# bioscan-ml/clibd

Hardware: AMD Instinct MI355X
Metric: paired samples/sec/step (I+D contrastive), global batch 2048 (higher is better)
Workload: dtype bf16

## Files before the change

clibd_amd/csrc/common.h:

```cpp
#pragma once
#include <hip/hip_runtime.h>
#include <stdint.h>

namespace clibd {

typedef __attribute__((ext_vector_type(8))) short bf16x8;
typedef __attribute__((ext_vector_type(4))) short bf16x4;
typedef __attribute__((ext_vector_type(4))) float f32x4;
typedef __attribute__((ext_vector_type(16))) float f32x16;
typedef __attribute__((address_space(3))) void lds_void;
typedef __attribute__((address_space(1))) const void gbl_cvoid;

__device__ __forceinline__ unsigned short f2bf(float x) {
    __bf16 h = (__bf16)x;
    return __builtin_bit_cast(unsigned short, h);
}
__device__ __forceinline__ float bf2f(unsigned short h) {
    return __builtin_bit_cast(float, ((unsigned)h) << 16);
}
__device__ __forceinline__ unsigned pack2bf(float lo, float hi) {
    typedef __bf16 bf16x2_t __attribute__((ext_vector_type(2)));
    typedef float f32x2_t __attribute__((ext_vector_type(2)));
    const bf16x2_t r = __builtin_convertvector((f32x2_t){lo, hi}, bf16x2_t);
    return __builtin_bit_cast(unsigned, r);
}
__device__ __forceinline__ float bfround(float x) { return bf2f(f2bf(x)); }

__device__ __forceinline__ unsigned pack4fp8(float a, float b, float c, float d) {
    a = __builtin_amdgcn_fmed3f(a, -448.f, 448.f); b = __builtin_amdgcn_fmed3f(b, -448.f, 448.f);
    c = __builtin_amdgcn_fmed3f(c, -448.f, 448.f); d = __builtin_amdgcn_fmed3f(d, -448.f, 448.f);
    int w = __builtin_amdgcn_cvt_pk_fp8_f32(a, b, 0, false);
    w = __builtin_amdgcn_cvt_pk_fp8_f32(c, d, w, true);
    return (unsigned)w;
}
__device__ __forceinline__ uint2 pack8fp8(const float v[8], float s) {
    uint2 o;
    o.x = pack4fp8(v[0] * s, v[1] * s, v[2] * s, v[3] * s);
    o.y = pack4fp8(v[4] * s, v[5] * s, v[6] * s, v[7] * s);
    return o;
}

__device__ __forceinline__ void glds16(const void* gsrc, void* lds_wave_base) {
    __builtin_amdgcn_global_load_lds((gbl_cvoid*)gsrc, (lds_void*)lds_wave_base, 16, 0, 0);
}

__device__ __forceinline__ void store16_stream(void* p, uint4 v) {
#ifdef CLIBD_NT_STORES
    typedef unsigned u32x4_t __attribute__((ext_vector_type(4)));
    __builtin_nontemporal_store((u32x4_t){v.x, v.y, v.z, v.w}, (u32x4_t*)p);
#else
    *(uint4*)p = v;
#endif
}

__device__ __forceinline__ unsigned drop_hash(unsigned seed, unsigned pair) {
    unsigned x = pair ^ seed;
    x ^= x >> 16; x *= 0x7feb352du; x ^= x >> 15; x *= 0x846ca68bu; x ^= x >> 16;
    return x;
}
__device__ __forceinline__ void drop_pair(unsigned seed, unsigned idx_even, unsigned thr16, float scale, float& f0, float& f1) {
    const unsigned h = drop_hash(seed, idx_even >> 1);
    f0 = (h & 0xffffu) >= thr16 ? scale : 0.f;
    f1 = (h >> 16) >= thr16 ? scale : 0.f;
}
__device__ __forceinline__ float drop_one(unsigned seed, unsigned idx, unsigned thr16, float scale) {
    const unsigned h = drop_hash(seed, idx >> 1);
    return (((idx & 1u) ? (h >> 16) : (h & 0xffffu)) >= thr16) ? scale : 0.f;
}

template <int CTRL>
__device__ __forceinline__ float dpp_mov(float v) {
    return __builtin_bit_cast(float, __builtin_amdgcn_update_dpp(0, __builtin_bit_cast(int, v), CTRL, 0xF, 0xF, false));
}
constexpr int DPP_QUAD_XOR1 = 0xB1, DPP_QUAD_XOR2 = 0x4E, DPP_ROW_HALF_MIRROR = 0x141, DPP_ROW_MIRROR = 0x140, DPP_ROW_ROR8 = 0x128;
__device__ __forceinline__ void permlane32_swap(float& a, float& b) {
    asm volatile("s_nop 1\n\tv_permlane32_swap_b32 %0, %1\n\ts_nop 1" : "+v"(a), "+v"(b));
}
__device__ __forceinline__ void permlane16_swap(float& a, float& b) {
    asm volatile("s_nop 1\n\tv_permlane16_swap_b32 %0, %1\n\ts_nop 1" : "+v"(a), "+v"(b));
}
__device__ __forceinline__ float rows4_sum(float v) {
    float a = v, b = v;
    permlane16_swap(a, b);
    v = a + b;
    a = v; b = v;
    permlane32_swap(a, b);
    return a + b;
}
__device__ __forceinline__ float rows4_max(float v) {
    float a = v, b = v;
    permlane16_swap(a, b);
    v = fmaxf(a, b);
    a = v; b = v;
    permlane32_swap(a, b);
    return fmaxf(a, b);
}
__device__ __forceinline__ float wave_sum(float v) {
    v += dpp_mov<DPP_QUAD_XOR1>(v);
    v += dpp_mov<DPP_QUAD_XOR2>(v);
    v += dpp_mov<DPP_ROW_HALF_MIRROR>(v);
    v += dpp_mov<DPP_ROW_MIRROR>(v);
    return rows4_sum(v);
}
__device__ __forceinline__ float wave_max(float v) {
    v = fmaxf(v, dpp_mov<DPP_QUAD_XOR1>(v));
    v = fmaxf(v, dpp_mov<DPP_QUAD_XOR2>(v));
    v = fmaxf(v, dpp_mov<DPP_ROW_HALF_MIRROR>(v));
    v = fmaxf(v, dpp_mov<DPP_ROW_MIRROR>(v));
    return rows4_max(v);
}

__device__ __forceinline__ float fast_erf(float x) {
    float ax = fabsf(x);
    float t = __builtin_amdgcn_rcpf(1.0f + 0.3275911f * ax);
    float y = ((((1.061405429f * t - 1.453152027f) * t + 1.421413741f) * t - 0.284496736f) * t + 0.254829592f) * t;
    float e = __expf(-ax * ax);
    float r = 1.0f - y * e;
    return copysignf(r, x);
}
__device__ __forceinline__ float gelu_f(float x) {
    return 0.5f * x * (1.0f + fast_erf(x * 0.70710678118654752f));
}
__device__ __forceinline__ void gelu_and_grad_f(float x, float& y, float& dy) {
    const float ax = fabsf(x) * 0.70710678118654752f;
    const float t = __builtin_amdgcn_rcpf(1.0f + 0.3275911f * ax);
    const float poly = ((((1.061405429f * t - 1.453152027f) * t + 1.421413741f) * t - 0.284496736f) * t + 0.254829592f) * t;
    const float e = __expf(-ax * ax);
    const float erfv = copysignf(1.0f - poly * e, x);
    const float cdf = 0.5f * (1.0f + erfv);
    y = x * cdf;
    dy = cdf + x * (0.3989422804014327f * e);
}
typedef float f32x2 __attribute__((ext_vector_type(2)));
__device__ __forceinline__ void gelu_and_grad_x2(f32x2 x, f32x2& y, f32x2& dy) {
    constexpr float K = 0.84932180028801907f;
    constexpr float P = 0.3275911f * 0.70710678118654752f / K;
    f32x2 ax = {fabsf(x[0]), fabsf(x[1])};
    ax = ax * K;
    const f32x2 d = ax * P + 1.0f;
    const f32x2 t = {__builtin_amdgcn_rcpf(d[0]), __builtin_amdgcn_rcpf(d[1])};
    const f32x2 poly = ((((0.5307027145f * t - 0.7265760135f) * t + 0.7107068705f) * t - 0.142248368f) * t + 0.127414796f) * t;
    const f32x2 s = ax * ax;
    const f32x2 e = {__builtin_amdgcn_exp2f(-s[0]), __builtin_amdgcn_exp2f(-s[1])};
    const f32x2 h = 0.5f - poly * e;
    const f32x2 hs = {copysignf(h[0], x[0]), copysignf(h[1], x[1])};
    const f32x2 cdf = hs + 0.5f;
    y = x * cdf;
    dy = (x * e) * 0.3989422804014327f + cdf;
}
__device__ __forceinline__ f32x2 bfround2(float a, float b) {
// ... 85 lines not shown
```

clibd_amd/csrc/gemm.hip:

```cpp
#include <stdlib.h>

#include <cmath>

#include "gemm_common.h"
#include "host_util.h"

namespace clibd {

constexpr int BM = 128, BN = 128, BK = 64;
constexpr int TILE_BYTES = BM * BK * 2;
constexpr int GEMM_THREADS = 256;

__device__ __forceinline__ int w_row_perm(int r) {
    const int r6 = r & 63;
    return (r & 64) + w_col_of(r6 >> 4, r6 & 15);
}

__global__ __launch_bounds__(GEMM_THREADS, 2) void gemm_bf16_nt_kernel(GemmParams p) {
    extern __shared__ __attribute__((aligned(16))) char smem[];
    const int tid = threadIdx.x;
    const int lane = tid & 63;
    const int wave = __builtin_amdgcn_readfirstlane(tid >> 6);
    const int wm = wave >> 1, wn = wave & 1;

// ... 25 lines not shown
#pragma unroll
    for (int i = 0; i < 4; ++i)
#pragma unroll
        for (int j = 0; j < 4; ++j) acc[i][j] = (f32x4){0.f, 0.f, 0.f, 0.f};

    const int frow = lane & 15, fch = lane >> 4;
    int a_off[4], w_off[4];
#pragma unroll
    for (int t = 0; t < 4; ++t) {
        const int ra = wm * 64 + t * 16 + frow;
        const int rw = wn * 64 + t * 16 + frow;
        a_off[t] = ra * 128 + ((fch ^ (ra & 7)) << 4);
        w_off[t] = rw * 128 + ((fch ^ (rw & 7)) << 4);
    }

    auto stage = [&](int kt, int buf) {
        char* base = smem + buf * (2 * TILE_BYTES);
        int kta = kt0 + kt;
        if (kta >= p.hole_kt) kta += p.hole_nkt;
        const size_t koff = (size_t)kta * (BK * 2);
#pragma unroll
        for (int j = 0; j < 4; ++j) {
            glds16(a_src[j] + koff, base + (wave * 4 + j) * 1024);
            glds16(w_src[j] + koff, base + TILE_BYTES + (wave * 4 + j) * 1024);
        }
    };

    if (nk > 0) stage(0, 0);
    for (int kt = 0; kt < nk; ++kt) {
        __syncthreads();
        if (kt + 1 < nk) stage(kt + 1, (kt + 1) & 1);
        const char* ab = smem + (kt & 1) * (2 * TILE_BYTES);
        const char* wb = ab + TILE_BYTES;
#pragma unroll
        for (int kk = 0; kk < 2; ++kk) {
            bf16x8 af[4], wf[4];
#pragma unroll
            for (int t = 0; t < 4; ++t) {
                af[t] = *(const bf16x8*)(ab + (a_off[t] ^ (kk << 6)));
                wf[t] = *(const bf16x8*)(wb + (w_off[t] ^ (kk << 6)));
            }
#pragma unroll
            for (int i = 0; i < 4; ++i)
#pragma unroll
                for (int j = 0; j < 4; ++j)
                    acc[i][j] = __builtin_amdgcn_mfma_f32_16x16x32_bf16(wf[j], af[i], acc[i][j], 0, 0, 0);
        }
    }

    const clibd_gemm_epilogue& ep = p.ep;
    if (ep.rank_u != nullptr && split == 0) {
        bf16x8 uf[4], vf[4];
#pragma unroll
        for (int t = 0; t < 4; ++t) {
            uf[t] = (bf16x8){0, 0, 0, 0, 0, 0, 0, 0};
            vf[t] = (bf16x8){0, 0, 0, 0, 0, 0, 0, 0};
            if (fch == 0) {
                const int gm = min(m0 + wm * 64 + t * 16 + frow, p.M - 1);
                const int gn = min(n0 + w_row_perm(wn * 64 + t * 16 + frow), p.N - 1);
                uf[t] = *(const bf16x8*)((const unsigned short*)ep.rank_u + (size_t)gm * ep.ld_rank_u);
                vf[t] = *(const bf16x8*)((const unsigned short*)ep.rank_v + (size_t)gn * 8);
            }
        }
#pragma unroll
        for (int i = 0; i < 4; ++i)
#pragma unroll
            for (int j = 0; j < 4; ++j)
                acc[i][j] = __builtin_amdgcn_mfma_f32_16x16x32_bf16(vf[j], uf[i], acc[i][j], 0, 0, 0);
    }

    const int nb = n0 + wn * 64 + 16 * fch;
    if (nb >= p.N) return;
    float bias[16];
    load_bias16(ep, nb, split == 0, bias);
#pragma unroll
    for (int i = 0; i < 4; ++i) {
        const int m = m0 + wm * 64 + 16 * i + frow;
        if (m >= p.M) continue;
        float v[16];
#pragma unroll
        for (int j = 0; j < 4; ++j)
#pragma unroll
            for (int r = 0; r < 4; ++r) v[4 * j + r] = acc[i][j][r] + bias[4 * j + r];
        store_row16(ep, m, nb, v);
    }
}

__global__ __launch_bounds__(256) void transpose_bf16_kernel(const unsigned short* in, int ld_in, int R, int C,
                                                             unsigned short* out, int ld_out) {
    __shared__ unsigned short tile[64][66];
    const int r0 = blockIdx.y * 64, c0 = blockIdx.x * 64;
    const int tx = threadIdx.x & 63, ty = threadIdx.x >> 6;
    for (int i = ty; i < 64; i += 4) {
        const int r = r0 + i, c = c0 + tx;
        tile[i][tx] = (r < R && c < C) ? in[(size_t)r * ld_in + c] : (unsigned short)0;
    }
    __syncthreads();
    for (int i = ty; i < 64; i += 4) {
        const int c = c0 + i, r = r0 + tx;
        if (c < C && r < ld_out) out[(size_t)c * ld_out + r] = tile[tx][i];
    }
}

__global__ __launch_bounds__(256) void transpose_fp8_bf16_kernel(const unsigned char* __restrict__ in, int ld_in, int R, int C, float scale,
                                                                 unsigned short* __restrict__ out, int ld_out) {
    __shared__ unsigned short tile[64][66];
    const int r0 = blockIdx.y * 64, c0 = blockIdx.x * 64;
    const int tx = threadIdx.x & 63, ty = threadIdx.x >> 6;
    for (int i = ty; i < 64; i += 4) {
        const int r = r0 + i, c = c0 + tx;
        unsigned short v = 0;
        if (r < R && c < C) v = f2bf(__builtin_amdgcn_cvt_f32_fp8((int)in[(size_t)r * ld_in + c], 0) * scale);
        tile[i][tx] = v;
    }
    __syncthreads();
    for (int i = ty; i < 64; i += 4) {
        const int c = c0 + i, r = r0 + tx;
        if (c < C && r < ld_out) out[(size_t)c * ld_out + r] = tile[tx][i];
    }
}

template <int RB>
__global__ __launch_bounds__(256) void transpose_colsum_bf16_kernel(const unsigned short* __restrict__ in, int ld_in, int R, int C,
                                                                    unsigned short* __restrict__ out, int ld_out,
                                                                    float* __restrict__ colsum, float* __restrict__ partials) {
    __shared__ __attribute__((aligned(16))) unsigned short tile[64 * RB * 66];
    const int r0 = blockIdx.y * (64 * RB), c0 = blockIdx.x * 64;
    const int t = threadIdx.x;
    uint4 v[2 * RB];
#pragma unroll
    for (int k = 0; k < 2 * RB; ++k) {
        const int row = (t >> 3) + 32 * k, ch = t & 7;
        v[k] = make_uint4(0u, 0u, 0u, 0u);
        if (r0 + row < R && c0 + 8 * ch < C) v[k] = *(const uint4*)(in + (size_t)(r0 + row) * ld_in + c0 + 8 * ch);
    }
#pragma unroll
    for (int k = 0; k < 2 * RB; ++k) {
        const int row = (t >> 3) + 32 * k, ch = t & 7;
        unsigned* d = (unsigned*)(tile + row * 66 + 8 * ch);
        d[0] = v[k].x; d[1] = v[k].y; d[2] = v[k].z; d[3] = v[k].w;
    }
    __syncthreads();
#pragma unroll
    for (int k = 0; k < 2; ++k) {
        const int c = (t >> 3) + 32 * k, rch = t & 7;
        float sum = 0.f;
#pragma unroll
        for (int rb = 0; rb < RB; ++rb) {
            unsigned short e[8];
#pragma unroll
            for (int j = 0; j < 8; ++j) e[j] = tile[(64 * rb + 8 * rch + j) * 66 + c];
            if (c0 + c < C && r0 + 64 * rb + 8 * rch < ld_out) {
                uint4 o;
                o.x = (unsigned)e[0] | ((unsigned)e[1] << 16); o.y = (unsigned)e[2] | ((unsigned)e[3] << 16);
                o.z = (unsigned)e[4] | ((unsigned)e[5] << 16); o.w = (unsigned)e[6] | ((unsigned)e[7] << 16);
                *(uint4*)(out + (size_t)(c0 + c) * ld_out + r0 + 64 * rb + 8 * rch) = o;
            }
            if (colsum != nullptr) {
#pragma unroll
                for (int j = 0; j < 8; ++j) sum += bf2f(e[j]);
            }
        }
        if (colsum != nullptr) {
            sum += dpp_mov<DPP_QUAD_XOR1>(sum);
            sum += dpp_mov<DPP_QUAD_XOR2>(sum);
            sum += dpp_mov<DPP_ROW_HALF_MIRROR>(sum);
            if (rch == 0 && c0 + c < C) {
// ... 35 lines not shown
            for (int k = 0; k < 8; ++k) v[k] = partials[(size_t)(b + k) * C + c];
#pragma unroll
            for (int k = 0; k < 8; ++k) s += v[k];
        }
        for (; b < b1; ++b) s += partials[(size_t)b * C + c];
    }
    part[w][lane] = s;
    __syncthreads();
    if (w == 0 && c < C) {
        float t = part[0][lane];
        for (int k = 1; k < G; ++k) t += part[k][lane];
        if (c < split) out[c] += t;
        else out_b[c - split] += t;
    }
}

int ordered_colsum_launch(const float* partials, int nblk, int C, float* out, int split, float* out_b, hipStream_t stream) {
    if (nblk <= 0 || C <= 0) return CLIBD_OK;
    const int G = nblk < 16 ? nblk : 16;
    hipLaunchKernelGGL(ordered_colsum_kernel, dim3((unsigned)((C + 63) / 64)), dim3(64 * G), 0, stream, partials, nblk, C, out, split, out_b);
    return check_launch("ordered_colsum");
}

__global__ __launch_bounds__(256) void cast_f32_bf16_kernel(const float* in, unsigned short* out, size_t n) {
    size_t i = ((size_t)blockIdx.x * blockDim.x + threadIdx.x) * 4;
    const size_t stride = (size_t)gridDim.x * blockDim.x * 4;
    for (; i + 3 < n; i += stride) {
        const f32x4 v = *(const f32x4*)(in + i);
        uint2 o;
        o.x = pack2bf(v[0], v[1]);
        o.y = pack2bf(v[2], v[3]);
        *(uint2*)(out + i) = o;
    }
    if (blockIdx.x == 0 && threadIdx.x == 0)
        for (size_t j = n & ~(size_t)3; j < n; ++j) out[j] = f2bf(in[j]);
}

__global__ __launch_bounds__(256) void cast_transpose_f32_bf16_kernel(const float* in, int R, int C,
                                                                      unsigned short* out) {
    __shared__ float tile[64][65];
    const int r0 = blockIdx.y * 64, c0 = blockIdx.x * 64;
    const int tx = threadIdx.x & 63, ty = threadIdx.x >> 6;
    for (int i = ty; i < 64; i += 4) {
        const int r = r0 + i, c = c0 + tx;
        tile[i][tx] = (r < R && c < C) ? in[(size_t)r * C + c] : 0.f;
    }
    __syncthreads();
    for (int i = ty; i < 64; i += 4) {
        const int c = c0 + i, r = r0 + tx;
        if (c < C && r < R) out[(size_t)c * R + r] = f2bf(tile[tx][i]);
    }
}

}

using namespace clibd;

static int gemm_impl(const void* A, int lda, const void* W, int ldw, int M, int N, int K, int hole_k0, int hole_len,
                     const clibd_gemm_epilogue* ep, void* tail_ws, size_t tail_ws_bytes, void* stream) {
    if (!A || !W || !ep) return set_error(CLIBD_EINVAL, "gemm: null pointer");
    if (hole_len < 0 || hole_k0 < 0 || hole_k0 % BK || hole_len % BK || hole_k0 + hole_len > K || (hole_len > 0 && hole_len >= K))
        return set_error(CLIBD_EINVAL, "gemm: bad K hole (multiples of 64 inside [0, K))");
    if (M <= 0 || N <= 0 || K <= 0) return set_error(CLIBD_EINVAL, "gemm: non-positive shape");
    if (K % BK != 0) return set_error(CLIBD_EINVAL, "gemm: K must be a multiple of 64");
    if (N % 16 != 0) return set_error(CLIBD_EINVAL, "gemm: N must be a multiple of 16");
    if (lda % 8 != 0 || ldw % 8 != 0 || lda < K || ldw < K) return set_error(CLIBD_EINVAL, "gemm: bad lda/ldw");
    if (!aligned16(A) || !aligned16(W)) return set_error(CLIBD_EINVAL, "gemm: operands must be 16-byte aligned");
    if (!ep->out_bf16 && !ep->out_f32 && !ep->out_pre_bf16) return set_error(CLIBD_EINVAL, "gemm: no output");
    if ((ep->rank_u == nullptr) != (ep->rank_v == nullptr)) return set_error(CLIBD_EINVAL, "gemm: rank_u/rank_v");
    if (ep->rank_u && (ep->ld_rank_u < 8 || ep->ld_rank_u % 8)) return set_error(CLIBD_EINVAL, "gemm: ld_rank_u");
    if ((ep->act == CLIBD_ACT_GELU_GRAD || ep->act == CLIBD_ACT_MUL_AUX || ep->act == CLIBD_ACT_ADD_AUX) &&
        (!ep->aux_bf16 || ep->ld_aux % 8 || ep->ld_aux < N))
        return set_error(CLIBD_EINVAL, "gemm: GELU_GRAD / MUL_AUX / ADD_AUX need aux_bf16 with ld_aux >= N, % 8");
    if (ep->act == CLIBD_ACT_MUL_AUX_U8 && (!ep->aux_bf16 || ep->ld_aux % 16 || ep->ld_aux < N))
        return set_error(CLIBD_EINVAL, "gemm: MUL_AUX_U8 needs aux (one byte per element) with ld_aux >= N, % 16");
    const bool e12 = ep->act == CLIBD_ACT_GELU_SAVE_GRAD_E12 || ep->act == CLIBD_ACT_MUL_AUX_E12;
    if (e12 && (N % 8 != 0)) return set_error(CLIBD_EINVAL, "gemm: the e4m7 gelu' forms need N % 8 == 0");
    if (ep->act == CLIBD_ACT_MUL_AUX_E12 && (!ep->aux_bf16 || ep->ld_aux % 4 || ep->ld_aux < 3 * (N / 2)))
        return set_error(CLIBD_EINVAL, "gemm: MUL_AUX_E12 needs aux (1.5 bytes per element) with ld_aux >= 3N/2 bytes, % 4");
    if (ep->act == CLIBD_ACT_GELU_SAVE_GRAD_E12 && (!ep->out_pre_bf16 || ep->ld_pre % 4 || ep->ld_pre < 3 * (N / 2)))
        return set_error(CLIBD_EINVAL, "gemm: GELU_SAVE_GRAD_E12 needs out_pre (1.5 bytes per element) with ld_pre >= 3N/2 bytes, % 4");
    if ((ep->act == CLIBD_ACT_GELU_SAVE_GRAD || ep->act == CLIBD_ACT_GELU_SAVE_GRAD_U8) && !ep->out_pre_bf16)
        return set_error(CLIBD_EINVAL, "gemm: GELU_SAVE_GRAD needs out_pre_bf16");
    if (ep->act < 0 || ep->act > CLIBD_ACT_MUL_AUX_E12) return set_error(CLIBD_EINVAL, "gemm: bad act");
    if (ep->residual_f32 && (ep->ld_res % 4 || ep->ld_res < N)) return set_error(CLIBD_EINVAL, "gemm: ld_res");
    if (ep->out_pre_bf16 && (ep->ld_pre % (ep->act == CLIBD_ACT_GELU_SAVE_GRAD_U8 ? 16 : 8) || ep->ld_pre < N)) return set_error(CLIBD_EINVAL, "gemm: ld_pre");
    if (ep->out_bf16 && (ep->ld_out_bf16 % 8 || ep->ld_out_bf16 < N)) return set_error(CLIBD_EINVAL, "gemm: ld_out_bf16");
    if (ep->out_f32 && (ep->ld_out_f32 % 4 || ep->ld_out_f32 < N)) return set_error(CLIBD_EINVAL, "gemm: ld_out_f32");
    if (ep->drop_thr16 < 0 || ep->drop_thr16 > 65535 || (ep->drop_thr16 > 0 && (ep->drop_ld < N || (ep->drop_ld & 1) || ep->split_k > 1)))
        return set_error(CLIBD_EINVAL, "gemm: bad dropout parameters");
    const int split = ep->split_k < 1 ? 1 : ep->split_k;
    if (split > 1 && (ep->out_bf16 || ep->out_pre_bf16 || ep->act != CLIBD_ACT_NONE || ep->residual_f32 || !ep->out_f32))
        return set_error(CLIBD_EINVAL, "gemm: split_k > 1 supports only a plain fp32 accumulate output");
    const void* ptrs[] = {ep->bias, ep->rank_u, ep->rank_v, ep->aux_bf16, ep->residual_f32, ep->out_pre_bf16,
                          ep->out_bf16, ep->out_f32};
    for (const void* q : ptrs)
        if (q && !aligned16(q)) return set_error(CLIBD_EINVAL, "gemm: epilogue pointers must be 16-byte aligned");

    GemmParams p{};
    p.A = (const unsigned short*)A; p.W = (const unsigned short*)W;
    p.M = M; p.N = N; p.K = K; p.lda = lda; p.ldw = ldw;
    p.tiles_m = (M + BM - 1) / BM;
    p.tiles_n = (N + BN - 1) / BN;
    const int ktiles = (K - hole_len) / BK;
    p.ktiles_per_split = (ktiles + split - 1) / split;
    p.ep = *ep;
    p.ep.split_k = split;
    p.splits = 1; p.nk_split = 0; p.split_stride = 0;
    p.hole_kt = hole_len > 0 ? hole_k0 / BK : 0x7fffffff;
    p.hole_nkt = hole_len / BK;
    const size_t tail_need = gemm256_tail_workspace_bytes(M, N, K);
    if (int e = check_workspace("gemm", "tail workspace", tail_ws, tail_ws_bytes, tail_need, "clibd_gemm_tail_workspace_bytes")) return e;
    if (tail_ws != nullptr && tail_need > 0) {
        p.sk_flags = (unsigned*)tail_ws;
        p.sk_ws = (float*)((char*)tail_ws + 1024);
    }
    static const int forced = [] { const char* e = getenv("CLIBD_GEMM_KERNEL"); return e ? atoi(e) : 0; }();
    const bool fold_epi = ep->row_sums != nullptr || ep->row_stats != nullptr;
    if (fold_epi) {
        if (epilogue_kind(p.ep) < 0)
            return set_error(CLIBD_EINVAL, "gemm: LN-fold epilogue: row_sums needs bias + residual_f32 + out_f32 + out_bf16 (act NONE); row_stats needs "
                                           "col_sum_w + bias + GELU_SAVE_GRAD with out_pre_bf16 + out_bf16; no rank update, dropout or split-K");
        if ((ep->row_sums && !aligned16(ep->row_sums)) || (ep->row_stats && !aligned16(ep->row_stats)) || (ep->col_sum_w && !aligned16(ep->col_sum_w)))
            return set_error(CLIBD_EINVAL, "gemm: LN-fold epilogue pointers must be 16-byte aligned");
        if (forced == 1 || hole_len != 0 || !gemm256_try_launch(p, (hipStream_t)stream))
            return set_error(CLIBD_EINVAL, "gemm: the LN-fold epilogues exist in the 256x256 kernel only (M >= 1024, N % 256 == 0, K % 128 == 0, >= 128 tiles)");
        return check_launch("gemm256_bf16_nt");
    }
    if (forced != 1 && hole_len == 0 && gemm256_try_launch(p, (hipStream_t)stream)) return check_launch("gemm256_bf16_nt");
    const long long nblocks = (long long)p.tiles_m * p.tiles_n * split;
    if (nblocks > 0x7fffffffLL) return set_error(CLIBD_EINVAL, "gemm: grid too large");
    static const bool attr_ok = [] {
        return hipFuncSetAttribute((const void*)gemm_bf16_nt_kernel, hipFuncAttributeMaxDynamicSharedMemorySize,
                                   4 * TILE_BYTES) == hipSuccess;
    }();
    (void)attr_ok;
    hipLaunchKernelGGL(gemm_bf16_nt_kernel, dim3((unsigned)nblocks), dim3(GEMM_THREADS), 4 * TILE_BYTES,
                       (hipStream_t)stream, p);
    return check_launch("gemm_bf16_nt");
}

extern "C" size_t clibd_gemm_tail_workspace_bytes(int M, int N, int K) { return gemm256_tail_workspace_bytes(M, N, K); }

extern "C" int clibd_gemm_bf16_nt(const void* A, int lda, const void* W, int ldw, int M, int N, int K,
                                  const clibd_gemm_epilogue* ep, void* workspace, size_t workspace_bytes, void* stream) {
    return gemm_impl(A, lda, W, ldw, M, N, K, 0, 0, ep, workspace, workspace_bytes, stream);
}

extern "C" int clibd_gemm_bf16_nt_khole(const void* A, int lda, const void* W, int ldw, int M, int N, int K, int hole_k0, int hole_len,
                                        const clibd_gemm_epilogue* ep, void* stream) {
    return gemm_impl(A, lda, W, ldw, M, N, K, hole_k0, hole_len, ep, nullptr, 0, stream);
}

extern "C" int clibd_gemm_fp8_nt(const void* A, int lda, const void* W, int ldw, int M, int N, int K, const float* col_scale,
                                 float out_fp8_scale, const clibd_gemm_epilogue* ep, void* stream) {
    if (!A || !W || !ep || !col_scale) return set_error(CLIBD_EINVAL, "gemm_fp8: null pointer");
    if (M <= 0 || N <= 0 || K <= 0 || lda < K || ldw < K) return set_error(CLIBD_EINVAL, "gemm_fp8: bad shape");
    if ((lda & 15) || (ldw & 15) || !aligned16(A) || !aligned16(W) || !aligned16(col_scale)) return set_error(CLIBD_EINVAL, "gemm_fp8: alignment (lda, ldw % 16)");
    if (ep->ld_out_bf16 & 7 || ep->ld_out_f32 & 3 || ep->ld_res & 3 || ep->ld_pre & 7 || ep->ld_rank_u & 7)
        return set_error(CLIBD_EINVAL, "gemm_fp8: leading dimensions");
    if ((ep->out_bf16 && !aligned16(ep->out_bf16)) || (ep->out_f32 && !aligned16(ep->out_f32)) || (ep->out_pre_bf16 && !aligned16(ep->out_pre_bf16)) ||
        (ep->residual_f32 && !aligned16(ep->residual_f32)) || (ep->rank_u && !aligned16(ep->rank_u)) || (ep->rank_v && !aligned16(ep->rank_v)) ||
        (ep->bias && !aligned16(ep->bias)))
        return set_error(CLIBD_EINVAL, "gemm_fp8: pointer alignment");
    if ((ep->rank_u == nullptr) != (ep->rank_v == nullptr)) return set_error(CLIBD_EINVAL, "gemm_fp8: rank_u / rank_v must come together");
    GemmParams p{};
    p.A = (const unsigned short*)A; p.W = (const unsigned short*)W;
    p.M = M; p.N = N; p.K = K; p.lda = lda; p.ldw = ldw;
    p.ep = *ep;
    if (p.ep.split_k < 1) p.ep.split_k = 1;
    p.fp8 = 1; p.col_scale = col_scale; p.out_fp8_scale = out_fp8_scale;
    if (!gemm256_fp8_launch(p, (hipStream_t)stream))
        return set_error(CLIBD_EINVAL, "gemm_fp8: shape / epilogue not supported (N % 256, K % 256, K >= 512, bias required; forms: "
                                       "[lora] bias->bf16 | bias->gelu->fp8 + gelu' | bias[->dropout]+residual->f32)");
    return check_launch("gemm256_fp8_nt");
}

extern "C" int clibd_gemm_fp8_dgrad_nt(const void* A, int lda, const void* W, int ldw, int M, int N, int K, const float* col_scale,
                                       const float* a_row_dequant, float out_fp8_scale, const clibd_gemm_epilogue* ep, void* stream) {
    if (!A || !W || !ep || !col_scale) return set_error(CLIBD_EINVAL, "gemm_fp8_dgrad: null pointer");
    if (M <= 0 || N <= 0 || K <= 0 || lda < K || ldw < K) return set_error(CLIBD_EINVAL, "gemm_fp8_dgrad: bad shape");
    if ((lda & 15) || (ldw & 15) || !aligned16(A) || !aligned16(W) || !aligned16(col_scale) || (a_row_dequant && !aligned16(a_row_dequant)))
        return set_error(CLIBD_EINVAL, "gemm_fp8_dgrad: alignment (lda, ldw % 16)");
    if (ep->ld_out_bf16 & 7 || ep->ld_aux & 7) return set_error(CLIBD_EINVAL, "gemm_fp8_dgrad: leading dimensions");
    if (ep->act == CLIBD_ACT_MUL_AUX_U8 && (!ep->aux_bf16 || ep->ld_aux % 16 || ep->ld_aux < N))
        return set_error(CLIBD_EINVAL, "gemm_fp8_dgrad: MUL_AUX_U8 needs aux (one byte per element) with ld_aux >= N, % 16");
    if (!ep->out_bf16 || !aligned16(ep->out_bf16) || (ep->aux_bf16 && !aligned16(ep->aux_bf16))) return set_error(CLIBD_EINVAL, "gemm_fp8_dgrad: out_bf16 / aux alignment");
    if (ep->out_f32 || ep->residual_f32 || ep->bias || ep->rank_u || ep->rank_v || ep->row_sums || ep->row_stats || ep->col_sum_w)
        return set_error(CLIBD_EINVAL, "gemm_fp8_dgrad: only out_bf16 [+ aux_bf16] epilogues");
    const bool mul_form = ep->act == CLIBD_ACT_MUL_AUX || ep->act == CLIBD_ACT_MUL_AUX_U8 || ep->act == CLIBD_ACT_MUL_AUX_E12;
    if (ep->act == CLIBD_ACT_MUL_AUX_E12 && (!ep->aux_bf16 || ep->ld_aux % 4 || ep->ld_aux < 3 * (N / 2)))
        return set_error(CLIBD_EINVAL, "gemm_fp8_dgrad: MUL_AUX_E12 needs aux (1.5 bytes per element) with ld_aux >= 3N/2 bytes, % 4");
    if (ep->out_pre_bf16 && (!mul_form || !a_row_dequant || !aligned16(ep->out_pre_bf16) || (ep->ld_pre & 7) || ep->ld_pre < N))
        return set_error(CLIBD_EINVAL, "gemm_fp8_dgrad: out_pre_bf16 (bf16 copy) comes with MUL_AUX[_U8] and a_row_dequant only; ld_pre >= N, % 8; 16-byte aligned");
    GemmParams p{};
    p.A = (const unsigned short*)A; p.W = (const unsigned short*)W;
    p.M = M; p.N = N; p.K = K; p.lda = lda; p.ldw = ldw;
    p.ep = *ep;
    if (p.ep.split_k < 1) p.ep.split_k = 1;
    p.fp8 = 1; p.col_scale = col_scale; p.out_fp8_scale = out_fp8_scale; p.a_row_dequant = a_row_dequant;
    p.dual_bf16 = (unsigned short*)p.ep.out_pre_bf16; p.ld_dual = p.ep.ld_pre;
// ... 172 lines not shown
```

clibd_amd/csrc/gemm256.hip:

```cpp
#include <cstdlib>
#include "gemm_common.h"
#include "host_util.h"

namespace clibd {

constexpr int T_M = 256, T_N = 256, T_K = 64;
constexpr int HALF_BYTES = 128 * T_K * 2;
constexpr int STAGE_BYTES = 4 * HALF_BYTES;
constexpr int G256_THREADS = 512;
constexpr int G256_LDS = 2 * STAGE_BYTES;
constexpr size_t G256_SK_FLAG_BYTES = 1024;
#ifndef CLIBD_WS_MIN_TILES_N
#define CLIBD_WS_MIN_TILES_N 1
#endif
#ifndef CLIBD_WS_GROUP
#define CLIBD_WS_GROUP 6
#endif
constexpr int G256_WS_MIN_TILES_N = CLIBD_WS_MIN_TILES_N, G256_WS_GROUP = CLIBD_WS_GROUP;

#define CLIBD_WAIT_VMCNT(n) asm volatile("s_waitcnt vmcnt(" #n ")" ::: "memory")

typedef int i32x8 __attribute__((ext_vector_type(8)));
typedef int i32x4 __attribute__((ext_vector_type(4)));
__device__ __forceinline__ i32x8 cat_frag(bf16x8 lo, bf16x8 hi) {
// ... 268 lines not shown
            for (int b = 0; b < 4; ++b)
#pragma unroll
                for (int c = 0; c < 2; ++c)
#pragma unroll
                    for (int d = 0; d < 2; ++d) acc[a][b][c][d] = (f32x4){0.f, 0.f, 0.f, 0.f};

        int kt = 0;
        PHASE_HEAD(0); PHASE_HEAD(1); PHASE_HEAD(2); PHASE_HEAD(3);
        STAMP(1);
        PHASE_HEAD(4); PHASE_HEAD(5);
        PHASE(6, true, 8); PHASE(7, true, 8);
        STAMP(2);
        for (kt = 2; kt < nk - 2; kt += 2) {
            PHASE(0, true, 8); PHASE(1, true, 8); PHASE(2, true, 8); PHASE(3, true, 8);
            PHASE(4, true, 8); PHASE(5, true, 8); PHASE(6, true, 8); PHASE(7, true, 8);
        }
        STAMP(3);
        PHASE(0, true, 8); PHASE(1, true, 8);
        if (has_next) set_sources(next);
        PHASE_TAIL(2, 6); PHASE_TAIL(3, 4); PHASE_TAIL(4, 2); PHASE_TAIL(5, 0); PHASE_TAIL(6, 0); PHASE_TAIL(7, 0);
        if (wm == 0) BARRIER();
        if constexpr (FP8) {
#pragma unroll
            for (int hm = 0; hm < 2; ++hm)
                asm volatile("s_nop 15\n\ts_nop 15"
                             : "+v"(acc[hm][0][0][0]), "+v"(acc[hm][0][0][1]), "+v"(acc[hm][0][1][0]), "+v"(acc[hm][0][1][1]),
                               "+v"(acc[hm][1][0][0]), "+v"(acc[hm][1][0][1]), "+v"(acc[hm][1][1][0]), "+v"(acc[hm][1][1][1]),
                               "+v"(acc[hm][2][0][0]), "+v"(acc[hm][2][0][1]), "+v"(acc[hm][2][1][0]), "+v"(acc[hm][2][1][1]),
                               "+v"(acc[hm][3][0][0]), "+v"(acc[hm][3][0][1]), "+v"(acc[hm][3][1][0]), "+v"(acc[hm][3][1][1])
                             :: "memory");
        }
        STAMP(4);
        if constexpr (SK) {
            if (slot_cur >= 0) {
                const int srow = 64 * wn + 4 * fch, scol = 128 * wm + 8 * frow;
                if (part_cur > 0) {
                    float* outp = p.sk_ws + ((size_t)(part_cur - 1) * (size_t)p.sk_tail + (size_t)slot_cur) * (size_t)(T_M * T_N);
#pragma unroll
                    for (int hn = 0; hn < 2; ++hn)
#pragma unroll
                        for (int n = 0; n < 2; ++n)
#pragma unroll
                            for (int r = 0; r < 4; ++r) {
                                float* o = outp + (size_t)(srow + 32 * hn + 16 * n + r) * T_N + scol;
                                const f32x4 v0 = (f32x4){acc[0][0][hn][n][r], acc[0][1][hn][n][r], acc[0][2][hn][n][r], acc[0][3][hn][n][r]};
                                const f32x4 v1 = (f32x4){acc[1][0][hn][n][r], acc[1][1][hn][n][r], acc[1][2][hn][n][r], acc[1][3][hn][n][r]};
                                asm volatile("global_store_dwordx4 %0, %1, off sc0 sc1\n\tglobal_store_dwordx4 %0, %2, off offset:16 sc0 sc1" :: "v"(o), "v"(v0), "v"(v1) : "memory");
                            }
                    asm volatile("s_waitcnt vmcnt(0)" ::: "memory");
                    BARRIER();
                    if (tid == 0) __hip_atomic_fetch_add(p.sk_flags + slot_cur, 1u, __ATOMIC_RELAXED, __HIP_MEMORY_SCOPE_AGENT);
                    break;
                }
                if (tid == 0) {
                    while (__hip_atomic_load(p.sk_flags + slot_cur, __ATOMIC_RELAXED, __HIP_MEMORY_SCOPE_AGENT) < (unsigned)(p.sk_parts - 1)) __builtin_amdgcn_s_sleep(16);
                    __hip_atomic_store(p.sk_flags + slot_cur, 0u, __ATOMIC_RELAXED, __HIP_MEMORY_SCOPE_AGENT);
                }
                BARRIER();
                for (int q = 1; q < p.sk_parts; ++q) {
                    const float* inp = p.sk_ws + ((size_t)(q - 1) * (size_t)p.sk_tail + (size_t)slot_cur) * (size_t)(T_M * T_N);
#pragma unroll
                    for (int hn = 0; hn < 2; ++hn)
#pragma unroll
                        for (int n = 0; n < 2; ++n) {
                            f32x4 t0[4], t1[4];
#pragma unroll
                            for (int r = 0; r < 4; ++r) {
                                const float* o = inp + (size_t)(srow + 32 * hn + 16 * n + r) * T_N + scol;
                                asm volatile("global_load_dwordx4 %0, %2, off sc0 sc1\n\tglobal_load_dwordx4 %1, %2, off offset:16 sc0 sc1" : "=&v"(t0[r]), "=&v"(t1[r]) : "v"(o) : "memory");
                            }
                            asm volatile("s_waitcnt vmcnt(0)" : "+v"(t0[0]), "+v"(t0[1]), "+v"(t0[2]), "+v"(t0[3]), "+v"(t1[0]), "+v"(t1[1]), "+v"(t1[2]), "+v"(t1[3]));
#pragma unroll
                            for (int r = 0; r < 4; ++r)
#pragma unroll
                                for (int t = 0; t < 4; ++t) { acc[0][t][hn][n][r] += t0[r][t]; acc[1][t][hn][n][r] += t1[r][t]; }
                        }
                }
            }
        }
        int erow = frow, egrp = fch;
        asm volatile("" : "+v"(erow), "+v"(egrp));
        int nb = n0 + 128 * wm + 8 * erow;
        int mb = m0 + 64 * wn + 4 * egrp;
        constexpr bool RES_KIND = (KIND == EPI_RES_F32 || KIND == EPI_RES_F32_DROP || KIND == EPI_RES_F32_COPY);
        constexpr bool TWO_PASS = (epi_aux_kind(KIND) || RES_KIND || KIND == EPI_ROWNORM_GELU);
        constexpr bool PRELOAD_ROWS = TWO_PASS && !LORA && !FP8;
        f32x4 bias_q[2];
        uint4 in_aux[8];
        f32x4 in_res[8][2];
        float2 in_st[8];
        f32x4 col_s[2];
#define GLOAD128(dst, ptr) asm volatile("global_load_dwordx4 %0, %1, off ; EPI_OPERAND_LOAD" : "=&v"(dst) : "v"(ptr) : "memory")
        constexpr bool BIAS_ASM = BIAS && !FP8;
        if constexpr (BIAS_ASM) {
            const float* bp = ep.bias + nb;
            GLOAD128(bias_q[0], bp);
            GLOAD128(bias_q[1], bp + 4);
        }
        if constexpr (PRELOAD_ROWS) {
#pragma unroll
            for (int n = 0; n < 2; ++n)
#pragma unroll
                for (int r = 0; r < 4; ++r) {
                    const int mc = min(mb + 16 * n + r, p.M - 1);
                    if constexpr (KIND == EPI_ROWNORM_GELU) {
                        in_st[4 * n + r] = *(const float2*)(ep.row_stats + (size_t)mc * 2);
                    } else if constexpr (KIND == EPI_MUL_AUX_U8) {
                        const uint2 c8 = *(const uint2*)((const unsigned char*)ep.aux_bf16 + (size_t)mc * ep.ld_aux + nb);
                        in_aux[4 * n + r] = make_uint4(c8.x, c8.y, 0u, 0u);
                    } else if constexpr (KIND == EPI_MUL_AUX_12) {
                        in_aux[4 * n + r] = load_aux12((const unsigned char*)ep.aux_bf16 + (size_t)mc * ep.ld_aux + (nb >> 1) * 3);
                    } else if constexpr (epi_aux_kind(KIND)) {
                        in_aux[4 * n + r] = load_aux16<epi_aux_nt(KIND)>((const unsigned short*)ep.aux_bf16 + (size_t)mc * ep.ld_aux + nb);
                    } else {
                        const f32x4* rs = (const f32x4*)(ep.residual_f32 + (size_t)mc * ep.ld_res + nb);
                        in_res[4 * n + r][0] = rs[0];
                        in_res[4 * n + r][1] = rs[1];
                    }
                }
        }
        if constexpr (KIND == EPI_ROWNORM_GELU) {
            col_s[0] = *(const f32x4*)(ep.col_sum_w + nb);
            col_s[1] = *(const f32x4*)(ep.col_sum_w + nb + 4);
        }
        if (has_next) {
            ISSUE(1, 2, 1); __builtin_amdgcn_sched_barrier(0);
            ISSUE(1, 3, 1); __builtin_amdgcn_sched_barrier(0);
        }
        erow = frow; egrp = fch;
        asm volatile("" : "+v"(erow), "+v"(egrp));
        nb = n0 + 128 * wm + 8 * erow;
        mb = m0 + 64 * wn + 4 * egrp;
#define EPI_TIED_WAIT(N)                                                                                             \
    do {                                                                                                             \
        if constexpr (BIAS_ASM) asm volatile("s_waitcnt vmcnt(" #N ") ; EPI_OPERAND_WAIT" : "+v"(bias_q[0]), "+v"(bias_q[1])); \
    } while (0)
        if constexpr (KIND == EPI_ROWNORM_GELU) {
            if (!has_next) asm volatile("s_waitcnt vmcnt(10)" ::: "memory");
            EPI_TIED_WAIT(14);
        } else if constexpr (PRELOAD_ROWS && epi_aux_kind(KIND)) {
            if (!has_next) asm volatile("s_waitcnt vmcnt(8)" ::: "memory");
            EPI_TIED_WAIT(12);
        } else if constexpr (PRELOAD_ROWS) {
            if (!has_next) asm volatile("s_waitcnt vmcnt(16)" ::: "memory");
            EPI_TIED_WAIT(20);
        } else {
            if (!has_next) asm volatile("s_waitcnt vmcnt(0)" ::: "memory");
            EPI_TIED_WAIT(4);
        }
#undef EPI_TIED_WAIT
#undef GLOAD128
        unsigned rdexp[2][2];
        if constexpr (FP8) {
            const float* csp = p.col_scale + n0 + 128 * wm + 8 * erow;
            const f32x4 c0 = *(const f32x4*)csp, c1 = *(const f32x4*)(csp + 4);
#pragma unroll
            for (int hm = 0; hm < 2; ++hm)
#pragma unroll
                for (int t = 0; t < 4; ++t) {
                    const float c = hm ? c1[t] : c0[t];
#pragma unroll
                    for (int q = 0; q < 4; ++q) acc[hm][t][q >> 1][q & 1] *= c;
                }
            if constexpr (DG == 2) {
#pragma unroll
                for (int hn = 0; hn < 2; ++hn)
#pragma unroll
                    for (int n = 0; n < 2; ++n) {
                        const f32x4 rd = *(const f32x4*)(p.a_row_dequant + min(mb + 32 * hn + 16 * n, p.M - 4));
                        rdexp[hn][n] = ((__float_as_uint(rd[0]) >> 23) & 0xffu) | (((__float_as_uint(rd[1]) >> 23) & 0xffu) << 8) |
                                       (((__float_as_uint(rd[2]) >> 23) & 0xffu) << 16) | (((__float_as_uint(rd[3]) >> 23) & 0xffu) << 24);
                    }
            }
            if constexpr (DG && !epi_mul_aux_kind(KIND)) {
#pragma unroll
                for (int hn = 0; hn < 2; ++hn)
#pragma unroll
                    for (int n = 0; n < 2; ++n) {
                        const f32x4 rd = *(const f32x4*)(p.a_row_dequant + min(mb + 32 * hn + 16 * n, p.M - 4));
#pragma unroll
                        for (int hm = 0; hm < 2; ++hm)
#pragma unroll
                            for (int t = 0; t < 4; ++t) acc[hm][t][hn][n] *= rd;
                    }
            }
        }
        if (LORA) {
            bf16x8 uf[2][2];
#pragma unroll
            for (int hn = 0; hn < 2; ++hn)
#pragma unroll
                for (int n = 0; n < 2; ++n) {
                    uf[hn][n] = (bf16x8){0, 0, 0, 0, 0, 0, 0, 0};
                    if (egrp == 0) {
                        const int gm = min(m0 + 64 * wn + 32 * hn + 16 * n + erow, p.M - 1);
                        uf[hn][n] = *(const bf16x8*)((const unsigned short*)ep.rank_u + (size_t)gm * ep.ld_rank_u);
                    }
                }
#pragma unroll
            for (int hm = 0; hm < 2; ++hm)
#pragma unroll
                for (int t = 0; t < 4; ++t) {
                    bf16x8 vf = (bf16x8){0, 0, 0, 0, 0, 0, 0, 0};
                    if (egrp == 0) {
                        const int gn = nb + 4 * hm + t;
                        vf = *(const bf16x8*)((const unsigned short*)ep.rank_v + (size_t)gn * 8);
                    }
#pragma unroll
                    for (int n = 0; n < 4; ++n)
                        acc[hm][t][n >> 1][n & 1] = __builtin_amdgcn_mfma_f32_16x16x32_bf16(uf[n >> 1][n & 1], vf, acc[hm][t][n >> 1][n & 1], 0, 0, 0);
                }
            __builtin_amdgcn_sched_barrier(0);
        }

        {
            float bias[8];
            if constexpr (BIAS_ASM) {
#pragma unroll
                for (int e = 0; e < 4; ++e) { bias[e] = bias_q[0][e]; bias[4 + e] = bias_q[1][e]; }
            } else if constexpr (BIAS) {
                load_bias8(ep, nb, bias);
                if constexpr (!TWO_PASS) {
#pragma unroll
                    for (int e = 0; e < 8; ++e) asm volatile("" : "+v"(bias[e]));
                }
            }
#define EPV(hm, t) (BIAS ? acc[hm][t][hn][n][r] + bias[4 * (hm) + (t)] : acc[hm][t][hn][n][r])
#define FOR_ROWS_HN(HN0, HN1, ...)                                                                           \
    _Pragma("unroll") for (int hn = (HN0); hn < (HN1); ++hn)                                                 \
        _Pragma("unroll") for (int n = 0; n < 2; ++n)                                                        \
            _Pragma("unroll") for (int r = 0; r < 4; ++r) {                                                  \
                const int m = mb + 32 * hn + 16 * n + r;                                                     \
                __VA_ARGS__                                                                                  \
            }
#define FOR_ROWS(...) FOR_ROWS_HN(0, 2, __VA_ARGS__)
#define PIN_GROUP(hn_)                                                                                       \
    _Pragma("unroll") for (int hm = 0; hm < 2; ++hm)                                                         \
        _Pragma("unroll") for (int t = 0; t < 4; ++t)                                                        \
            _Pragma("unroll") for (int n2 = 0; n2 < 2; ++n2) asm volatile("" : "+v"(acc[hm][t][hn_][n2]))
            if (KIND == EPI_SPLITK_F32) {
                float* outp = ep.out_f32 + (size_t)split_cur * (size_t)p.split_stride;
                FOR_ROWS({
                    if (m < p.M) {
                        f32x4* o = (f32x4*)(outp + (size_t)m * ep.ld_out_f32 + nb);
                        o[0] = (f32x4){acc[0][0][hn][n][r], acc[0][1][hn][n][r], acc[0][2][hn][n][r], acc[0][3][hn][n][r]};
                        o[1] = (f32x4){acc[1][0][hn][n][r], acc[1][1][hn][n][r], acc[1][2][hn][n][r], acc[1][3][hn][n][r]};
                    }
                })
            } else if (TWO_PASS) {
                float cs8[8];
                if constexpr (KIND == EPI_ROWNORM_GELU) {
                    _Pragma("unroll") for (int e = 0; e < 4; ++e) { cs8[e] = col_s[0][e]; cs8[4 + e] = col_s[1][e]; }
                }
                FOR_ROWS_HN(0, 1, {
                    const int mc = min(m, p.M - 1);
                    float v[8];
                    _Pragma("unroll") for (int hm = 0; hm < 2; ++hm)
                        _Pragma("unroll") for (int t = 0; t < 4; ++t) v[4 * hm + t] = (KIND == EPI_ROWNORM_GELU) ? acc[hm][t][hn][n][r] : EPV(hm, t);
                    if constexpr (KIND == EPI_ROWNORM_GELU) fold_rownorm8(v, in_st[4 * n + r].x, in_st[4 * n + r].y, cs8, bias);
                    else if constexpr (PRELOAD_ROWS) fold_row8_in<KIND>(ep, mc, nb, v, in_aux[4 * n + r], in_res[4 * n + r][0], in_res[4 * n + r][1]);
                    else fold_row8<KIND>(ep, mc, nb, v);
                    _Pragma("unroll") for (int hm = 0; hm < 2; ++hm)
                        _Pragma("unroll") for (int t = 0; t < 4; ++t) acc[hm][t][hn][n][r] = v[4 * hm + t];
                })
                PIN_GROUP(0);
                FOR_ROWS_HN(1, 2, {
                    const int mc = min(m, p.M - 1);
                    float v[8];
                    _Pragma("unroll") for (int hm = 0; hm < 2; ++hm)
                        _Pragma("unroll") for (int t = 0; t < 4; ++t) v[4 * hm + t] = (KIND == EPI_ROWNORM_GELU) ? acc[hm][t][hn][n][r] : EPV(hm, t);
                    if constexpr (KIND == EPI_ROWNORM_GELU) {
                        const float2 st = *(const float2*)(ep.row_stats + (size_t)mc * 2);
                        fold_rownorm8(v, st.x, st.y, cs8, bias);
                    } else {
                        fold_row8<KIND>(ep, mc, nb, v);
                    }
                    _Pragma("unroll") for (int hm = 0; hm < 2; ++hm)
                        _Pragma("unroll") for (int t = 0; t < 4; ++t) acc[hm][t][hn][n][r] = v[4 * hm + t];
                })
                PIN_GROUP(1);
                float keep1 = 0.f, keep2 = 0.f;
                FOR_ROWS({
                    if (m < p.M) {
                        float v[8];
                        _Pragma("unroll") for (int hm = 0; hm < 2; ++hm)
                            _Pragma("unroll") for (int t = 0; t < 4; ++t) v[4 * hm + t] = acc[hm][t][hn][n][r];
                        if (KIND == EPI_ROWNORM_GELU) {
                            store_row8<EPI_GELU_SAVE>(ep, m, nb, v);
                        } else if (DG && epi_mul_aux_kind(KIND)) {
                            *(uint2*)((unsigned char*)ep.out_bf16 + (size_t)m * ep.ld_out_bf16 + nb) = pack8fp8(v, p.out_fp8_scale);
                            if constexpr (DG == 2) {
                                const float rdf = __uint_as_float(((rdexp[hn][n] >> (8 * r)) & 0xffu) << 23);
                                float w8[8];
                                _Pragma("unroll") for (int e = 0; e < 8; ++e) w8[e] = v[e] * rdf;
                                *(uint4*)(p.dual_bf16 + (size_t)m * p.ld_dual + nb) = pack8bf(w8);
                            }
                        } else if (epi_aux_kind(KIND)) {
                            *(uint4*)((unsigned short*)ep.out_bf16 + (size_t)m * ep.ld_out_bf16 + nb) = pack8bf(v);
                        } else {
                            f32x4* o = (f32x4*)(ep.out_f32 + (size_t)m * ep.ld_out_f32 + nb);
                            o[0] = (f32x4){v[0], v[1], v[2], v[3]};
                            o[1] = (f32x4){v[4], v[5], v[6], v[7]};
                            if constexpr (KIND == EPI_RES_F32_COPY) {
                                *(uint4*)((unsigned short*)ep.out_bf16 + (size_t)m * ep.ld_out_bf16 + nb) = pack8bf(v);
                                float s1 = ((v[0] + v[1]) + (v[2] + v[3])) + ((v[4] + v[5]) + (v[6] + v[7]));
                                float s2 = 0.f;
                                _Pragma("unroll") for (int e = 0; e < 8; ++e) s2 = fmaf(v[e], v[e], s2);
                                s1 = row16_sum(s1);
                                s2 = row16_sum(s2);
                                if (erow == 8 * hn + 4 * n + r) { keep1 = s1; keep2 = s2; }
                            }
                        }
                    }
                })
                if constexpr (KIND == EPI_RES_F32_COPY) {
                    const int jm = mb + 32 * (erow >> 3) + 16 * ((erow >> 2) & 1) + (erow & 3);
                    const int slice = (n0 >> 7) + wm;
                    if (jm < p.M) *(float2*)(ep.row_sums + ((size_t)slice * (size_t)p.M + (size_t)jm) * 2) = make_float2(keep1, keep2);
                }
            } else {
                FOR_ROWS({
                    if (m < p.M) {
                        float v[8];
                        _Pragma("unroll") for (int hm = 0; hm < 2; ++hm)
                            _Pragma("unroll") for (int t = 0; t < 4; ++t) v[4 * hm + t] = EPV(hm, t);
                        if (FP8 && KIND == EPI_GELU_SAVE) store_row8_gelu_fp8(ep, m, nb, v, p.out_fp8_scale);
                        else store_row8<KIND>(ep, m, nb, v);
                    }
                })
            }
#undef PIN_GROUP
#undef FOR_ROWS_HN
#undef FOR_ROWS
#undef EPV
        }
        STAMP(5);
        if (DIAG) ++tile_i;
        if (!has_next) break;
        allow_case = (m0 + T_M <= p.M) ? stores_case : 0;
        tile = next;
    }
}

template <int KIND, bool LORA, bool BIAS, bool DIAG, bool FP8>
__global__ __launch_bounds__(G256_THREADS) void gemm256_bf16_nt_kernel(GemmParams p, int ntiles, int skew_ticks, long long* stamps) {
    gemm256_body<KIND, LORA, BIAS, DIAG, FP8, 0>(p, ntiles, skew_ticks, stamps);
}
template <int KIND, bool LORA, bool BIAS>
__global__ __launch_bounds__(G256_THREADS) void gemm256_bf16_nt_sk_kernel(GemmParams p, int ntiles, int skew_ticks, long long* stamps) {
    gemm256_body<KIND, LORA, BIAS, false, false, 0, true>(p, ntiles, skew_ticks, stamps);
}
static const void* kernel_ptr_sk(int kind, bool lora, bool bias) {
    switch (kind) {
        case EPI_BF16: return bias ? nullptr : lora ? (const void*)gemm256_bf16_nt_sk_kernel<EPI_BF16, true, false> : (const void*)gemm256_bf16_nt_sk_kernel<EPI_BF16, false, false>;
        case EPI_ADD_AUX: return bias ? nullptr : lora ? (const void*)gemm256_bf16_nt_sk_kernel<EPI_ADD_AUX, true, false> : (const void*)gemm256_bf16_nt_sk_kernel<EPI_ADD_AUX, false, false>;
        case EPI_RES_F32: return (bias && !lora) ? (const void*)gemm256_bf16_nt_sk_kernel<EPI_RES_F32, false, true> : nullptr;
        case EPI_RES_F32_DROP: return (bias && !lora) ? (const void*)gemm256_bf16_nt_sk_kernel<EPI_RES_F32_DROP, false, true> : nullptr;
        default: return nullptr;
    }
}
template <int KIND, int DG = 1>
__global__ __launch_bounds__(G256_THREADS) void gemm256_fp8_dgrad_kernel(GemmParams p, int ntiles, int skew_ticks, long long* stamps) {
    gemm256_body<KIND, false, false, false, true, DG>(p, ntiles, skew_ticks, stamps);
}

#ifdef CLIBD_GEMM_DIAG
static long long* g_stamp_buffer = nullptr;
static int skew_env_value() {
    static const int v = [] { const char* e = getenv("CLIBD_GEMM_SKEW"); return e ? atoi(e) : 0; }();
    return v;
}
static int band_env_value() {
    static const int v = [] { const char* e = getenv("CLIBD_GEMM_BAND"); return e ? atoi(e) : 0; }();
    return v;
}
#define CLIBD_DIAG_KERNEL(KIND) (const void*)gemm256_bf16_nt_kernel<KIND, false, true, true, false>
#else
static constexpr long long* g_stamp_buffer = nullptr;
static int skew_env_value() { return 0; }
static int band_env_value() { return 0; }
#define CLIBD_DIAG_KERNEL(KIND) (const void*)nullptr
#endif

static const void* kernel_ptr(int kind, bool lora, bool bias, bool diag) {
#define K256(KIND)                                                                                                    \
    (diag ? CLIBD_DIAG_KERNEL(KIND)                                                                                   \
          : lora ? (bias ? (const void*)gemm256_bf16_nt_kernel<KIND, true, true, false, false>                        \
                         : (const void*)gemm256_bf16_nt_kernel<KIND, true, false, false, false>)                      \
                 : (bias ? (const void*)gemm256_bf16_nt_kernel<KIND, false, true, false, false>                       \
                         : (const void*)gemm256_bf16_nt_kernel<KIND, false, false, false, false>))
    switch (kind) {
        case EPI_BF16: return K256(EPI_BF16);
        case EPI_GELU_SAVE: return K256(EPI_GELU_SAVE);
        case EPI_GELU: return K256(EPI_GELU);
        case EPI_F32: return K256(EPI_F32);
        case EPI_MUL_AUX: return K256(EPI_MUL_AUX);
        case EPI_ADD_AUX: return K256(EPI_ADD_AUX);
        case EPI_GELU_SAVE_U8: return K256(EPI_GELU_SAVE_U8);
        case EPI_MUL_AUX_U8: return K256(EPI_MUL_AUX_U8);
        case EPI_GELU_SAVE_12: return K256(EPI_GELU_SAVE_12);
        case EPI_MUL_AUX_12: return K256(EPI_MUL_AUX_12);
        case EPI_RES_F32: return K256(EPI_RES_F32);
        case EPI_RES_F32_DROP: return K256(EPI_RES_F32_DROP);
        case EPI_SPLITK_F32: return (const void*)gemm256_bf16_nt_kernel<EPI_SPLITK_F32, false, false, false, false>;
        case EPI_RES_F32_COPY: return (lora || !bias || diag) ? nullptr : (const void*)gemm256_bf16_nt_kernel<EPI_RES_F32_COPY, false, true, false, false>;
        case EPI_ROWNORM_GELU: return (lora || !bias || diag) ? nullptr : (const void*)gemm256_bf16_nt_kernel<EPI_ROWNORM_GELU, false, true, false, false>;
        default: return K256(EPI_GENERIC);
    }
#undef K256
}

static const void* kernel_ptr_fp8(int kind, bool lora) {
    switch (kind) {
        case EPI_BF16: return lora ? (const void*)gemm256_bf16_nt_kernel<EPI_BF16, true, true, false, true>
                                   : (const void*)gemm256_bf16_nt_kernel<EPI_BF16, false, true, false, true>;
        case EPI_GELU_SAVE: return lora ? nullptr : (const void*)gemm256_bf16_nt_kernel<EPI_GELU_SAVE, false, true, false, true>;
        case EPI_RES_F32: return lora ? nullptr : (const void*)gemm256_bf16_nt_kernel<EPI_RES_F32, false, true, false, true>;
        case EPI_RES_F32_DROP: return lora ? nullptr : (const void*)gemm256_bf16_nt_kernel<EPI_RES_F32_DROP, false, true, false, true>;
        default: return nullptr;
    }
}

static int device_cus() {
    static const int num_cus = [] {
        int dev = 0, n = 256;
        if (hipGetDevice(&dev) == hipSuccess) {
            hipDeviceProp_t prop;
            if (hipGetDeviceProperties(&prop, dev) == hipSuccess && prop.multiProcessorCount > 0) n = prop.multiProcessorCount;
        }
        return n;
    }();
    return num_cus;
}

bool gemm256_fp8_launch(const GemmParams& p, hipStream_t stream) {
    const int nk = p.K / 128;
    if (!p.fp8 || p.col_scale == nullptr || p.K % 128 != 0 || nk < 4 || (nk & 1) || p.N % T_N != 0 || p.M < 1 || p.ep.split_k > 1) return false;
    if (p.ep.bias == nullptr) return false;
    if ((unsigned long long)p.M * p.lda >= (1ull << 32) || (unsigned long long)p.N * p.ldw >= (1ull << 32)) return false;
    const int kind = epilogue_kind(p.ep);
    const bool lora = p.ep.rank_u != nullptr;
    const void* fn = kernel_ptr_fp8(kind, lora);
    if (fn == nullptr) return false;
    if ((p.out_fp8_scale > 0.f) != (kind == EPI_GELU_SAVE)) return false;
    static const bool attr_ok = [] {
        bool ok = true;
        for (int k = 0; k < EPI_NUM_KINDS; ++k)
            for (int l = 0; l < 2; ++l) {
                const void* f = kernel_ptr_fp8(k, l != 0);
                if (f != nullptr) ok = ok && hipFuncSetAttribute(f, hipFuncAttributeMaxDynamicSharedMemorySize, G256_LDS) == hipSuccess;
            }
        return ok;
    }();
    if (!attr_ok) return false;
    GemmParams q = p;
    q.tiles_m = (p.M + T_M - 1) / T_M;
    q.tiles_n = p.N / T_N;
    q.splits = 1;
    q.nk_split = nk;
    q.split_stride = 0;
    q.band = q.tiles_n >= G256_WS_MIN_TILES_N ? -G256_WS_GROUP : 4;
    const long long tiles = (long long)q.tiles_m * q.tiles_n;
    const int grid = (int)(tiles < device_cus() ? tiles : device_cus());
    int ntiles_i = (int)tiles, skew = 0;
    long long* stamp = nullptr;
    void* args[] = {(void*)&q, (void*)&ntiles_i, (void*)&skew, (void*)&stamp};
    return hipLaunchKernel(fn, dim3((unsigned)grid), dim3(G256_THREADS), args, G256_LDS, stream) == hipSuccess;
}

bool gemm256_fp8_dgrad_launch(const GemmParams& p, hipStream_t stream) {
    const int nk = p.K / 128;
    if (!p.fp8 || p.col_scale == nullptr || p.K % 128 != 0 || nk < 4 || (nk & 1) || p.N % T_N != 0 || p.M < 4 || (p.M & 3) || p.ep.split_k > 1) return false;
    if (p.ep.bias != nullptr || p.ep.rank_u != nullptr || p.ep.drop_thr16 > 0) return false;
    if ((unsigned long long)p.M * p.lda >= (1ull << 32) || (unsigned long long)p.N * p.ldw >= (1ull << 32)) return false;
    const int kind = epilogue_kind(p.ep);
    const bool dual = p.dual_bf16 != nullptr;
    const void* fn = kind == EPI_BF16 ? (const void*)gemm256_fp8_dgrad_kernel<EPI_BF16>
                   : kind == EPI_MUL_AUX ? (dual ? (const void*)gemm256_fp8_dgrad_kernel<EPI_MUL_AUX, 2> : (const void*)gemm256_fp8_dgrad_kernel<EPI_MUL_AUX>)
                   : kind == EPI_MUL_AUX_U8 ? (dual ? (const void*)gemm256_fp8_dgrad_kernel<EPI_MUL_AUX_U8, 2> : (const void*)gemm256_fp8_dgrad_kernel<EPI_MUL_AUX_U8>)
                   : kind == EPI_MUL_AUX_12 ? (dual ? (const void*)gemm256_fp8_dgrad_kernel<EPI_MUL_AUX_12, 2> : (const void*)gemm256_fp8_dgrad_kernel<EPI_MUL_AUX_12>)
                   : kind == EPI_ADD_AUX ? (const void*)gemm256_fp8_dgrad_kernel<EPI_ADD_AUX> : nullptr;
    if (fn == nullptr) return false;
    const bool mul = epi_mul_aux_kind(kind);
    if ((p.out_fp8_scale > 0.f) != mul) return false;
    if ((!mul || dual) && p.a_row_dequant == nullptr) return false;
    if (dual && (!mul || (p.ld_dual & 7) || p.ld_dual < p.N || ((uintptr_t)p.dual_bf16 & 15))) return false;
    static const bool attr_ok = [] {
        bool ok = hipFuncSetAttribute((const void*)gemm256_fp8_dgrad_kernel<EPI_BF16>, hipFuncAttributeMaxDynamicSharedMemorySize, G256_LDS) == hipSuccess;
        ok = ok && hipFuncSetAttribute((const void*)gemm256_fp8_dgrad_kernel<EPI_MUL_AUX>, hipFuncAttributeMaxDynamicSharedMemorySize, G256_LDS) == hipSuccess;
// ... 156 lines not shown
```

clibd_amd/csrc/gemm_common.h:

```cpp
#pragma once
#include "common.h"
#include "../../include/clibd_hip.h"

namespace clibd {

struct GemmParams {
    const unsigned short* A;
    const unsigned short* W;
    int M, N, K, lda, ldw;
    int tiles_m, tiles_n, ktiles_per_split;
    clibd_gemm_epilogue ep;
    int splits, nk_split;
    long long split_stride;
    int band;
    int hole_kt, hole_nkt;
    int fp8;
    const float* col_scale;
    float out_fp8_scale;
    const float* a_row_dequant;
    unsigned short* dual_bf16;
    int ld_dual;
    int sk_parts, sk_tail, sk_first, sk_nk_part;
    float* sk_ws;
    unsigned* sk_flags;
};

struct SkPlan { int parts, tail, first, nk_part; };
inline SkPlan plan_stream_k_tail(long long tiles, int num_cus, int nk) {
    SkPlan s{0, 0, 0, 0};
    if (tiles <= 0 || num_cus <= 0 || nk < 24 || (nk & 1)) return s;
    const long long full = (tiles / num_cus) * num_cus;
    const int tail = (int)(tiles - full);
    if (tail == 0 || 2 * tail > num_cus) return s;
    int P = num_cus / tail;
    if (P > 4) P = 4;
    for (; P >= 2; --P) {
        int nkp = (nk + P - 1) / P;
        nkp += nkp & 1;
        if (nkp < 4) nkp = 4;
        const int parts = (nk + nkp - 1) / nkp;
        const int last = nk - (parts - 1) * nkp;
        if (parts >= 2 && last >= 4 && (long long)parts * tail <= num_cus) { s.parts = parts; s.tail = tail; s.first = (int)full; s.nk_part = nkp; return s; }
    }
    return s;
}

__device__ __forceinline__ int w_col_of(int t, int i) { return 16 * (i >> 2) + 4 * t + (i & 3); }

__device__ __forceinline__ int tile_off(int row, int chunk) { return row * 128 + ((chunk ^ (row & 7)) << 4); }

__device__ __forceinline__ void tile_coords(int bid, int tiles_m, int tiles_n, int band, int& tile_m, int& tile_n) {
    const int ntiles = tiles_m * tiles_n;
    const int q = ntiles >> 3, r = ntiles & 7;
    const int xcd = bid & 7, idx = bid >> 3;
    bid = (xcd < r ? xcd * (q + 1) : r * (q + 1) + (xcd - r) * q) + idx;
    if (band < 0) {
        const int G = -band;
        const int g = bid / (tiles_m * G);
        const int rem = bid - g * tiles_m * G;
        const int gw = min(G, tiles_n - g * G);
        tile_m = rem / gw;
        tile_n = g * G + rem - tile_m * gw;
        return;
    }
    const int band_id = bid / (band * tiles_n);
    const int band_m0 = band_id * band;
    const int band_h = min(band, tiles_m - band_m0);
    const int in_band = bid - band_id * band * tiles_n;
    tile_m = band_m0 + in_band % band_h;
    tile_n = in_band / band_h;
}

__device__ __forceinline__ void load_bias16(const clibd_gemm_epilogue& ep, int nb, bool on, float bias[16]) {
#pragma unroll
    for (int e = 0; e < 16; ++e) bias[e] = 0.f;
    if (ep.bias != nullptr && on) {
#pragma unroll
        for (int q = 0; q < 4; ++q) {
            const f32x4 b4 = *(const f32x4*)(ep.bias + nb + 4 * q);
            bias[4 * q + 0] = b4[0]; bias[4 * q + 1] = b4[1]; bias[4 * q + 2] = b4[2]; bias[4 * q + 3] = b4[3];
        }
    }
}

__device__ __forceinline__ void store_row16(const clibd_gemm_epilogue& ep, int m, int nb, float v[16]) {
    if (ep.split_k > 1) {
        float* o = ep.out_f32 + (size_t)m * ep.ld_out_f32 + nb;
#pragma unroll
        for (int e = 0; e < 16; ++e) atomicAdd(o + e, v[e]);
        return;
    }
    if (ep.drop_thr16 > 0) {
        const unsigned base = (unsigned)m * (unsigned)ep.drop_ld + (unsigned)nb;
#pragma unroll
        for (int e = 0; e < 16; e += 2) {
            float f0, f1;
            drop_pair(ep.drop_seed, base + e, (unsigned)ep.drop_thr16, ep.drop_scale, f0, f1);
            v[e] *= f0;
            v[e + 1] *= f1;
        }
    }
    if (ep.act == CLIBD_ACT_GELU_SAVE_GRAD_E12) {
        float dg[16];
        gelu_and_grad_rows<16>(v, dg);
        gelu12_row8* o = (gelu12_row8*)((unsigned char*)ep.out_pre_bf16 + (size_t)m * ep.ld_pre + (nb >> 1) * 3);
        o[0] = gelu12_pack8(dg);
        o[1] = gelu12_pack8(dg + 8);
    } else if (ep.act == CLIBD_ACT_GELU_SAVE_GRAD_U8) {
        float dg[16];
        gelu_and_grad_rows<16>(v, dg);
        uint4 c;
        c.x = geluq_pack4(dg[0], dg[1], dg[2], dg[3]);   c.y = geluq_pack4(dg[4], dg[5], dg[6], dg[7]);
        c.z = geluq_pack4(dg[8], dg[9], dg[10], dg[11]); c.w = geluq_pack4(dg[12], dg[13], dg[14], dg[15]);
        store16_stream((unsigned char*)ep.out_pre_bf16 + (size_t)m * ep.ld_pre + nb, c);
    } else if (ep.act == CLIBD_ACT_GELU_SAVE_GRAD) {
        float dg[16];
        gelu_and_grad_rows<16>(v, dg);
        uint4 lo, hi;
        lo.x = pack2bf(dg[0], dg[1]);   lo.y = pack2bf(dg[2], dg[3]);   lo.z = pack2bf(dg[4], dg[5]);   lo.w = pack2bf(dg[6], dg[7]);
        hi.x = pack2bf(dg[8], dg[9]);   hi.y = pack2bf(dg[10], dg[11]); hi.z = pack2bf(dg[12], dg[13]); hi.w = pack2bf(dg[14], dg[15]);
        uint4* o = (uint4*)((unsigned short*)ep.out_pre_bf16 + (size_t)m * ep.ld_pre + nb);
        store16_stream(o, lo); store16_stream(o + 1, hi);
    } else if (ep.out_pre_bf16 != nullptr) {
        uint4 lo, hi;
        lo.x = pack2bf(v[0], v[1]);   lo.y = pack2bf(v[2], v[3]);   lo.z = pack2bf(v[4], v[5]);   lo.w = pack2bf(v[6], v[7]);
        hi.x = pack2bf(v[8], v[9]);   hi.y = pack2bf(v[10], v[11]); hi.z = pack2bf(v[12], v[13]); hi.w = pack2bf(v[14], v[15]);
        uint4* o = (uint4*)((unsigned short*)ep.out_pre_bf16 + (size_t)m * ep.ld_pre + nb);
        store16_stream(o, lo); store16_stream(o + 1, hi);
#pragma unroll
        for (int e = 0; e < 16; ++e) v[e] = bfround(v[e]);
    }
    if (ep.act == CLIBD_ACT_GELU) {
        gelu_rows<16>(v);
    } else if (ep.act == CLIBD_ACT_GELU_GRAD) {
        const uint4* ax = (const uint4*)((const unsigned short*)ep.aux_bf16 + (size_t)m * ep.ld_aux + nb);
        const uint4 x0 = ax[0], x1 = ax[1];
        const unsigned xs[8] = {x0.x, x0.y, x0.z, x0.w, x1.x, x1.y, x1.z, x1.w};
#pragma unroll
        for (int e = 0; e < 8; ++e) {
            v[2 * e] *= gelu_grad_f(bf2f((unsigned short)(xs[e] & 0xffffu)));
            v[2 * e + 1] *= gelu_grad_f(bf2f((unsigned short)(xs[e] >> 16)));
        }
    }
    if (ep.act == CLIBD_ACT_MUL_AUX_E12) {
        const gelu12_row8* ax = (const gelu12_row8*)((const unsigned char*)ep.aux_bf16 + (size_t)m * ep.ld_aux + (nb >> 1) * 3);
        const gelu12_row8 a0 = ax[0], a1 = ax[1];
        float d[16];
        gelu12_unpack8(a0.w0, a0.w1, a0.w2, d);
        gelu12_unpack8(a1.w0, a1.w1, a1.w2, d + 8);
#pragma unroll
        for (int e = 0; e < 16; ++e) v[e] *= d[e];
    }
    if (ep.act == CLIBD_ACT_MUL_AUX_U8) {
        const uint4 c = *(const uint4*)((const unsigned char*)ep.aux_bf16 + (size_t)m * ep.ld_aux + nb);
        const unsigned cs[4] = {c.x, c.y, c.z, c.w};
#pragma unroll
        for (int q = 0; q < 4; ++q) {
            float d[4];
            geluq_unpack4(cs[q], d);
            v[4 * q] *= d[0]; v[4 * q + 1] *= d[1]; v[4 * q + 2] *= d[2]; v[4 * q + 3] *= d[3];
        }
    }
    if (ep.act == CLIBD_ACT_MUL_AUX || ep.act == CLIBD_ACT_ADD_AUX) {
        const uint4* ax = (const uint4*)((const unsigned short*)ep.aux_bf16 + (size_t)m * ep.ld_aux + nb);
        const uint4 x0 = ax[0], x1 = ax[1];
        const unsigned xs[8] = {x0.x, x0.y, x0.z, x0.w, x1.x, x1.y, x1.z, x1.w};
#pragma unroll
        for (int e = 0; e < 8; ++e) {
            const float a0 = bf2f((unsigned short)(xs[e] & 0xffffu)), a1 = bf2f((unsigned short)(xs[e] >> 16));
            if (ep.act == CLIBD_ACT_MUL_AUX) { v[2 * e] *= a0; v[2 * e + 1] *= a1; }
            else { v[2 * e] += a0; v[2 * e + 1] += a1; }
        }
    }
    if (ep.residual_f32 != nullptr) {
        const f32x4* rs = (const f32x4*)(ep.residual_f32 + (size_t)m * ep.ld_res + nb);
#pragma unroll
        for (int q = 0; q < 4; ++q) {
            const f32x4 r4 = rs[q];
            v[4 * q + 0] += r4[0]; v[4 * q + 1] += r4[1]; v[4 * q + 2] += r4[2]; v[4 * q + 3] += r4[3];
        }
    }
    if (ep.out_f32 != nullptr) {
        f32x4* o = (f32x4*)(ep.out_f32 + (size_t)m * ep.ld_out_f32 + nb);
#pragma unroll
        for (int q = 0; q < 4; ++q) store16_stream(o + q, __builtin_bit_cast(uint4, (f32x4){v[4 * q], v[4 * q + 1], v[4 * q + 2], v[4 * q + 3]}));
    }
    if (ep.out_bf16 != nullptr) {
        uint4 lo, hi;
        lo.x = pack2bf(v[0], v[1]);   lo.y = pack2bf(v[2], v[3]);   lo.z = pack2bf(v[4], v[5]);   lo.w = pack2bf(v[6], v[7]);
        hi.x = pack2bf(v[8], v[9]);   hi.y = pack2bf(v[10], v[11]); hi.z = pack2bf(v[12], v[13]); hi.w = pack2bf(v[14], v[15]);
        uint4* o = (uint4*)((unsigned short*)ep.out_bf16 + (size_t)m * ep.ld_out_bf16 + nb);
        store16_stream(o, lo); store16_stream(o + 1, hi);
    }
}

__device__ __forceinline__ void load_bias8(const clibd_gemm_epilogue& ep, int nb, float bias[8]) {
#pragma unroll
    for (int e = 0; e < 8; ++e) bias[e] = 0.f;
    if (ep.bias != nullptr) {
        const f32x4 b0 = *(const f32x4*)(ep.bias + nb), b1 = *(const f32x4*)(ep.bias + nb + 4);
        bias[0] = b0[0]; bias[1] = b0[1]; bias[2] = b0[2]; bias[3] = b0[3];
        bias[4] = b1[0]; bias[5] = b1[1]; bias[6] = b1[2]; bias[7] = b1[3];
    }
}

__device__ __forceinline__ uint4 pack8bf(const float v[8]) {
    uint4 o;
    o.x = pack2bf(v[0], v[1]); o.y = pack2bf(v[2], v[3]); o.z = pack2bf(v[4], v[5]); o.w = pack2bf(v[6], v[7]);
    return o;
}

enum : int {
    EPI_GENERIC = 0,
    EPI_BF16 = 1,
    EPI_GELU_SAVE = 2,
    EPI_MUL_AUX = 3,
    EPI_RES_F32 = 4,
    EPI_RES_F32_DROP = 5,
    EPI_SPLITK_F32 = 6,
    EPI_ADD_AUX = 7,
    EPI_GELU_SAVE_U8 = 8,
    EPI_MUL_AUX_U8 = 9,
    EPI_RES_F32_COPY = 10,
    EPI_ROWNORM_GELU = 11,
    EPI_GELU_SAVE_12 = 12,
    EPI_MUL_AUX_12 = 13,
    EPI_GELU = 14,
    EPI_F32 = 15,
    EPI_NUM_KINDS = 16,
};
constexpr bool epi_aux_kind(int kind) { return kind == EPI_MUL_AUX || kind == EPI_ADD_AUX || kind == EPI_MUL_AUX_U8 || kind == EPI_MUL_AUX_12; }
constexpr bool epi_mul_aux_kind(int kind) { return kind == EPI_MUL_AUX || kind == EPI_MUL_AUX_U8 || kind == EPI_MUL_AUX_12; }

__host__ __device__ inline int epilogue_kind(const clibd_gemm_epilogue& ep) {
    if (ep.split_k > 1) return EPI_GENERIC;
    const bool drop = ep.drop_thr16 > 0;
    if (ep.row_sums != nullptr)
        return (ep.act == CLIBD_ACT_NONE && !drop && !ep.out_pre_bf16 && ep.residual_f32 && ep.out_f32 && ep.out_bf16 && !ep.rank_u && ep.bias) ? EPI_RES_F32_COPY : -1;
    if (ep.row_stats != nullptr)
        return (ep.act == CLIBD_ACT_GELU_SAVE_GRAD && !drop && ep.out_pre_bf16 && !ep.residual_f32 && !ep.out_f32 && ep.out_bf16 && !ep.rank_u && ep.bias && ep.col_sum_w) ? EPI_ROWNORM_GELU : -1;
    if (ep.act == CLIBD_ACT_NONE && !drop && !ep.out_pre_bf16 && !ep.residual_f32 && !ep.out_f32 && ep.out_bf16) return EPI_BF16;
    if (ep.act == CLIBD_ACT_GELU_SAVE_GRAD && !drop && ep.out_pre_bf16 && !ep.residual_f32 && !ep.out_f32 && ep.out_bf16) return EPI_GELU_SAVE;
    if (ep.act == CLIBD_ACT_GELU && !drop && !ep.out_pre_bf16 && !ep.residual_f32 && !ep.out_f32 && ep.out_bf16) return EPI_GELU;
    if (ep.act == CLIBD_ACT_MUL_AUX && !drop && !ep.out_pre_bf16 && !ep.residual_f32 && !ep.out_f32 && ep.out_bf16 && ep.aux_bf16) return EPI_MUL_AUX;
    if (ep.act == CLIBD_ACT_ADD_AUX && !drop && !ep.out_pre_bf16 && !ep.residual_f32 && !ep.out_f32 && ep.out_bf16 && ep.aux_bf16) return EPI_ADD_AUX;
    if (ep.act == CLIBD_ACT_GELU_SAVE_GRAD_U8 && !drop && ep.out_pre_bf16 && !ep.residual_f32 && !ep.out_f32 && ep.out_bf16) return EPI_GELU_SAVE_U8;
    if (ep.act == CLIBD_ACT_MUL_AUX_U8 && !drop && !ep.out_pre_bf16 && !ep.residual_f32 && !ep.out_f32 && ep.out_bf16 && ep.aux_bf16) return EPI_MUL_AUX_U8;
    if (ep.act == CLIBD_ACT_GELU_SAVE_GRAD_E12 && !drop && ep.out_pre_bf16 && !ep.residual_f32 && !ep.out_f32 && ep.out_bf16) return EPI_GELU_SAVE_12;
    if (ep.act == CLIBD_ACT_MUL_AUX_E12 && !drop && !ep.out_pre_bf16 && !ep.residual_f32 && !ep.out_f32 && ep.out_bf16 && ep.aux_bf16) return EPI_MUL_AUX_12;
    if (ep.act == CLIBD_ACT_GELU_SAVE_GRAD_E12 || ep.act == CLIBD_ACT_MUL_AUX_E12) return -1;
    if (ep.act == CLIBD_ACT_NONE && !ep.out_pre_bf16 && ep.residual_f32 && ep.out_f32 && !ep.out_bf16) return drop ? EPI_RES_F32_DROP : EPI_RES_F32;
    if (ep.act == CLIBD_ACT_NONE && !drop && !ep.out_pre_bf16 && !ep.residual_f32 && ep.out_f32 && !ep.out_bf16) return EPI_F32;
    return EPI_GENERIC;
}

template <int KIND>
__device__ __forceinline__ void store_row8(const clibd_gemm_epilogue& ep, int m, int nb, float v[8]) {
    if (KIND == EPI_BF16) {
        *(uint4*)((unsigned short*)ep.out_bf16 + (size_t)m * ep.ld_out_bf16 + nb) = pack8bf(v);
        return;
    }
    if (KIND == EPI_F32) {
        f32x4* o = (f32x4*)(ep.out_f32 + (size_t)m * ep.ld_out_f32 + nb);
        o[0] = (f32x4){v[0], v[1], v[2], v[3]};
        o[1] = (f32x4){v[4], v[5], v[6], v[7]};
        return;
    }
    if (KIND == EPI_GELU) {
        gelu_rows<8>(v);
        *(uint4*)((unsigned short*)ep.out_bf16 + (size_t)m * ep.ld_out_bf16 + nb) = pack8bf(v);
        return;
    }
    if (KIND == EPI_GELU_SAVE) {
        float dg[8];
        gelu_and_grad_rows<8>(v, dg);
        *(uint4*)((unsigned short*)ep.out_pre_bf16 + (size_t)m * ep.ld_pre + nb) = pack8bf(dg);
        *(uint4*)((unsigned short*)ep.out_bf16 + (size_t)m * ep.ld_out_bf16 + nb) = pack8bf(v);
        return;
    }
    if (KIND == EPI_GELU_SAVE_U8) {
        float dg[8];
        gelu_and_grad_rows<8>(v, dg);
        *(uint2*)((unsigned char*)ep.out_pre_bf16 + (size_t)m * ep.ld_pre + nb) =
            make_uint2(geluq_pack4(dg[0], dg[1], dg[2], dg[3]), geluq_pack4(dg[4], dg[5], dg[6], dg[7]));
        *(uint4*)((unsigned short*)ep.out_bf16 + (size_t)m * ep.ld_out_bf16 + nb) = pack8bf(v);
        return;
    }
    if (KIND == EPI_MUL_AUX_U8) {
        const uint2 c = *(const uint2*)((const unsigned char*)ep.aux_bf16 + (size_t)m * ep.ld_aux + nb);
        float d0[4], d1[4];
        geluq_unpack4(c.x, d0);
        geluq_unpack4(c.y, d1);
#pragma unroll
        for (int e = 0; e < 4; ++e) { v[e] *= d0[e]; v[4 + e] *= d1[e]; }
        *(uint4*)((unsigned short*)ep.out_bf16 + (size_t)m * ep.ld_out_bf16 + nb) = pack8bf(v);
        return;
    }
    if (KIND == EPI_GELU_SAVE_12) {
        float dg[8];
        gelu_and_grad_rows<8>(v, dg);
        *(gelu12_row8*)((unsigned char*)ep.out_pre_bf16 + (size_t)m * ep.ld_pre + (nb >> 1) * 3) = gelu12_pack8(dg);
        *(uint4*)((unsigned short*)ep.out_bf16 + (size_t)m * ep.ld_out_bf16 + nb) = pack8bf(v);
        return;
    }
    if (KIND == EPI_MUL_AUX_12) {
        const gelu12_row8 a = *(const gelu12_row8*)((const unsigned char*)ep.aux_bf16 + (size_t)m * ep.ld_aux + (nb >> 1) * 3);
        float d[8];
        gelu12_unpack8(a.w0, a.w1, a.w2, d);
#pragma unroll
        for (int e = 0; e < 8; ++e) v[e] *= d[e];
        *(uint4*)((unsigned short*)ep.out_bf16 + (size_t)m * ep.ld_out_bf16 + nb) = pack8bf(v);
        return;
    }
    if (KIND == EPI_MUL_AUX || KIND == EPI_ADD_AUX) {
        const uint4 x0 = *(const uint4*)((const unsigned short*)ep.aux_bf16 + (size_t)m * ep.ld_aux + nb);
        const unsigned xs[4] = {x0.x, x0.y, x0.z, x0.w};
#pragma unroll
        for (int e = 0; e < 4; ++e) {
            const float a0 = bf2f((unsigned short)(xs[e] & 0xffffu)), a1 = bf2f((unsigned short)(xs[e] >> 16));
// ... 22 lines not shown
            *(uint2*)((unsigned char*)ep.out_pre_bf16 + (size_t)m * ep.ld_pre + nb) =
                make_uint2(geluq_pack4(dg[0], dg[1], dg[2], dg[3]), geluq_pack4(dg[4], dg[5], dg[6], dg[7]));
        } else if (ep.act == CLIBD_ACT_GELU_SAVE_GRAD) {
            float dg[8];
            gelu_and_grad_rows<8>(v, dg);
            *(uint4*)((unsigned short*)ep.out_pre_bf16 + (size_t)m * ep.ld_pre + nb) = pack8bf(dg);
        } else if (ep.out_pre_bf16 != nullptr) {
            *(uint4*)((unsigned short*)ep.out_pre_bf16 + (size_t)m * ep.ld_pre + nb) = pack8bf(v);
#pragma unroll
            for (int e = 0; e < 8; ++e) v[e] = bfround(v[e]);
        }
        if (ep.act == CLIBD_ACT_GELU) {
            gelu_rows<8>(v);
        } else if (ep.act == CLIBD_ACT_MUL_AUX_U8) {
            const uint2 c = *(const uint2*)((const unsigned char*)ep.aux_bf16 + (size_t)m * ep.ld_aux + nb);
            float d0[4], d1[4];
            geluq_unpack4(c.x, d0);
            geluq_unpack4(c.y, d1);
#pragma unroll
            for (int e = 0; e < 4; ++e) { v[e] *= d0[e]; v[4 + e] *= d1[e]; }
        } else if (ep.act == CLIBD_ACT_GELU_GRAD || ep.act == CLIBD_ACT_MUL_AUX || ep.act == CLIBD_ACT_ADD_AUX) {
            const uint4 x0 = *(const uint4*)((const unsigned short*)ep.aux_bf16 + (size_t)m * ep.ld_aux + nb);
            const unsigned xs[4] = {x0.x, x0.y, x0.z, x0.w};
#pragma unroll
            for (int e = 0; e < 4; ++e) {
                const float a0 = bf2f((unsigned short)(xs[e] & 0xffffu)), a1 = bf2f((unsigned short)(xs[e] >> 16));
                if (ep.act == CLIBD_ACT_GELU_GRAD) {
                    v[2 * e] *= gelu_grad_f(a0);
                    v[2 * e + 1] *= gelu_grad_f(a1);
                } else if (ep.act == CLIBD_ACT_MUL_AUX) {
                    v[2 * e] *= a0;
                    v[2 * e + 1] *= a1;
                } else {
                    v[2 * e] += a0;
                    v[2 * e + 1] += a1;
                }
            }
        }
    }
    if (KIND == EPI_RES_F32 || KIND == EPI_RES_F32_DROP || ep.residual_f32 != nullptr) {
        const f32x4* rs = (const f32x4*)(ep.residual_f32 + (size_t)m * ep.ld_res + nb);
        const f32x4 r0 = rs[0], r1 = rs[1];
        v[0] += r0[0]; v[1] += r0[1]; v[2] += r0[2]; v[3] += r0[3];
        v[4] += r1[0]; v[5] += r1[1]; v[6] += r1[2]; v[7] += r1[3];
    }
    if (KIND == EPI_RES_F32 || KIND == EPI_RES_F32_DROP || ep.out_f32 != nullptr) {
        f32x4* o = (f32x4*)(ep.out_f32 + (size_t)m * ep.ld_out_f32 + nb);
        o[0] = (f32x4){v[0], v[1], v[2], v[3]};
        o[1] = (f32x4){v[4], v[5], v[6], v[7]};
    }
    if (KIND == EPI_GENERIC && ep.out_bf16 != nullptr) *(uint4*)((unsigned short*)ep.out_bf16 + (size_t)m * ep.ld_out_bf16 + nb) = pack8bf(v);
}

__device__ __forceinline__ void store_row8_gelu_fp8(const clibd_gemm_epilogue& ep, int m, int nb, float v[8], float out_scale) {
    float dg[8];
    gelu_and_grad_rows<8>(v, dg);
    *(uint4*)((unsigned short*)ep.out_pre_bf16 + (size_t)m * ep.ld_pre + nb) = pack8bf(dg);
    *(uint2*)((unsigned char*)ep.out_bf16 + (size_t)m * ep.ld_out_bf16 + nb) = pack8fp8(v, out_scale);
}

template <int KIND>
__device__ __forceinline__ void fold_row8_in(const clibd_gemm_epilogue& ep, int m, int nb, float v[8], const uint4& ax, const f32x4& r0,
                                             const f32x4& r1) {
    if (KIND == EPI_MUL_AUX_U8) {
        float d0[4], d1[4];
        geluq_unpack4(ax.x, d0);
        geluq_unpack4(ax.y, d1);
#pragma unroll
        for (int e = 0; e < 4; ++e) { v[e] *= d0[e]; v[4 + e] *= d1[e]; }
    } else if (KIND == EPI_MUL_AUX_12) {
        float d[8];
        gelu12_unpack8(ax.x, ax.y, ax.z, d);
#pragma unroll
        for (int e = 0; e < 8; ++e) v[e] *= d[e];
    } else if (KIND == EPI_MUL_AUX || KIND == EPI_ADD_AUX) {
        const unsigned xs[4] = {ax.x, ax.y, ax.z, ax.w};
#pragma unroll
        for (int e = 0; e < 4; ++e) {
            const float a0 = bf2f((unsigned short)(xs[e] & 0xffffu)), a1 = bf2f((unsigned short)(xs[e] >> 16));
            if (KIND == EPI_MUL_AUX) { v[2 * e] *= a0; v[2 * e + 1] *= a1; }
            else { v[2 * e] += a0; v[2 * e + 1] += a1; }
        }
    } else {
        if (KIND == EPI_RES_F32_DROP) {
            const unsigned base = (unsigned)m * (unsigned)ep.drop_ld + (unsigned)nb;
#pragma unroll
            for (int e = 0; e < 8; e += 2) {
                float f0, f1;
                drop_pair(ep.drop_seed, base + e, (unsigned)ep.drop_thr16, ep.drop_scale, f0, f1);
                v[e] *= f0;
                v[e + 1] *= f1;
            }
        }
        v[0] += r0[0]; v[1] += r0[1]; v[2] += r0[2]; v[3] += r0[3];
        v[4] += r1[0]; v[5] += r1[1]; v[6] += r1[2]; v[7] += r1[3];
    }
}

__device__ __forceinline__ void fold_rownorm8(float v[8], float mean, float rstd, const float s[8], const float b[8]) {
#pragma unroll
    for (int e = 0; e < 8; ++e) v[e] = fmaf(rstd, fmaf(-mean, s[e], v[e]), b[e]);
}

__device__ __forceinline__ float row16_sum(float x) {
    x += dpp_mov<DPP_QUAD_XOR1>(x);
    x += dpp_mov<DPP_QUAD_XOR2>(x);
    x += dpp_mov<DPP_ROW_HALF_MIRROR>(x);
    x += dpp_mov<DPP_ROW_MIRROR>(x);
    return x;
}

template <bool NT>
__device__ __forceinline__ uint4 load_aux16(const void* p) {
    typedef unsigned aux_u32x4 __attribute__((ext_vector_type(4)));
#ifndef CLIBD_PLAIN_AUX_LOADS
    const aux_u32x4 v = NT ? __builtin_nontemporal_load((const aux_u32x4*)p) : *(const aux_u32x4*)p;
#else
    const aux_u32x4 v = *(const aux_u32x4*)p;
#endif
    return make_uint4(v[0], v[1], v[2], v[3]);
}
#ifndef CLIBD_NT_ADD_AUX
#define CLIBD_NT_ADD_AUX 0
#endif
constexpr bool epi_aux_nt(int kind) { return kind != EPI_ADD_AUX || CLIBD_NT_ADD_AUX; }

__device__ __forceinline__ uint4 load_aux12(const void* p) {
    typedef unsigned aux_u32x3 __attribute__((ext_vector_type(3), aligned(4)));
#ifndef CLIBD_PLAIN_AUX_LOADS
    const aux_u32x3 v = __builtin_nontemporal_load((const aux_u32x3*)p);
#else
    const aux_u32x3 v = *(const aux_u32x3*)p;
#endif
    return make_uint4(v[0], v[1], v[2], 0u);
}

template <int KIND>
__device__ __forceinline__ void fold_row8(const clibd_gemm_epilogue& ep, int m, int nb, float v[8]) {
    uint4 ax = make_uint4(0u, 0u, 0u, 0u);
    f32x4 r0 = (f32x4){0.f, 0.f, 0.f, 0.f}, r1 = r0;
    if (KIND == EPI_MUL_AUX_U8) {
        const uint2 c = *(const uint2*)((const unsigned char*)ep.aux_bf16 + (size_t)m * ep.ld_aux + nb);
        ax.x = c.x; ax.y = c.y;
    } else if (KIND == EPI_MUL_AUX_12) {
        ax = load_aux12((const unsigned char*)ep.aux_bf16 + (size_t)m * ep.ld_aux + (nb >> 1) * 3);
    } else if (KIND == EPI_MUL_AUX || KIND == EPI_ADD_AUX) {
        ax = load_aux16<epi_aux_nt(KIND)>((const unsigned short*)ep.aux_bf16 + (size_t)m * ep.ld_aux + nb);
    } else {
        const f32x4* rs = (const f32x4*)(ep.residual_f32 + (size_t)m * ep.ld_res + nb);
        r0 = rs[0];
        r1 = rs[1];
    }
    fold_row8_in<KIND>(ep, m, nb, v, ax, r0, r1);
}

inline int plan_k_slices(int nk, int tiles, int num_cus, int* nks_out) {
    int splits = num_cus / (tiles > 0 ? tiles : 1);
    if (splits < 1) splits = 1;
    if (splits > nk / 4) splits = nk / 4;
    if (splits < 1) splits = 1;
    int nks = (nk + splits - 1) / splits;
    nks += nks & 1;
    if (nks < 4) nks = 4;
    if (nks > nk) nks = nk;
    splits = (nk + nks - 1) / nks;
    while (nk - (splits - 1) * nks < 4 && nks < nk) {
        nks += 2;
        if (nks > nk) nks = nk;
        splits = (nk + nks - 1) / nks;
    }
    *nks_out = nks;
    return splits;
}

bool gemm256_try_launch(const GemmParams& p, hipStream_t stream);
size_t gemm256_tail_workspace_bytes(int M, int N, int K);
bool gemm256_fp8_launch(const GemmParams& p, hipStream_t stream);
bool gemm256_fp8_dgrad_launch(const GemmParams& p, hipStream_t stream);
int gemm256_splitk_launch(const GemmParams& p, float* partials, size_t partials_elems, hipStream_t stream);

int gemm256_tn_splitk_launch(const unsigned short* A, int lda, const void* B, int ldb, int M, int Na, int Nb, float* partials,
                             size_t partials_elems, float* colsum, hipStream_t stream, float* colsum_partials, float b_scale);

}
```

clibd_amd/csrc/layernorm.hip:

```cpp
#include "common.h"
#include "../../include/clibd_hip.h"
#include "host_util.h"

namespace clibd {

constexpr int LN_MAX_CHUNKS = 4;

__device__ __forceinline__ float wave_reduce8(float v[8], int lane) {
    float w4[4], w2[2];
#pragma unroll
    for (int i = 0; i < 4; ++i) {
        float a = v[i], b = v[i + 4];
        permlane32_swap(a, b);
        w4[i] = a + b;
    }
#pragma unroll
    for (int i = 0; i < 2; ++i) {
        float a = w4[i], b = w4[i + 2];
        permlane16_swap(a, b);
        w2[i] = a + b;
    }
    const bool b3 = lane & 8;
    const float keep = b3 ? w2[1] : w2[0];
    const float send = b3 ? w2[0] : w2[1];
    float w1 = keep + dpp_mov<DPP_ROW_ROR8>(send);
    w1 += dpp_mov<DPP_ROW_HALF_MIRROR>(w1);
    w1 += dpp_mov<DPP_QUAD_XOR1>(w1);
    w1 += dpp_mov<DPP_QUAD_XOR2>(w1);
    return w1;
}

template <int NCH, bool LORA, int ROWS>
__global__ __launch_bounds__(256) void layernorm_fwd_kernel(const float* __restrict__ x, int M, int H,
                                                            const float* __restrict__ gamma,
                                                            const float* __restrict__ beta, float eps,
                                                            unsigned short* __restrict__ y_bf16,
                                                            float* __restrict__ y_f32, float* __restrict__ stats,
                                                            const unsigned short* __restrict__ lora_a,
                                                            unsigned short* __restrict__ t_bf16, unsigned drop_seed,
                                                            int drop_thr16, float drop_scale,
                                                            unsigned char* __restrict__ y_fp8, float fp8_scale) {
    extern __shared__ __attribute__((aligned(16))) float a_lds[];
    const int lane = threadIdx.x & 63;
    const int wave_in_grid = blockIdx.x * 4 + (threadIdx.x >> 6);
    const int nwaves = gridDim.x * 4;
    if (LORA) {
        for (int i = threadIdx.x; i < 8 * H; i += 256) a_lds[i] = bf2f(lora_a[i]);
        __syncthreads();
    }
    f32x4 g[NCH], b[NCH];
    bool act[NCH];
#pragma unroll
    for (int j = 0; j < NCH; ++j) {
        const int c = 4 * (lane + 64 * j);
        act[j] = c < H;
        g[j] = act[j] ? *(const f32x4*)(gamma + c) : (f32x4){0, 0, 0, 0};
        b[j] = act[j] ? *(const f32x4*)(beta + c) : (f32x4){0, 0, 0, 0};
    }
    const float invH = 1.0f / (float)H;
    for (int row0 = wave_in_grid * ROWS; row0 < M; row0 += nwaves * ROWS) {
        f32x4 v[ROWS][NCH];
        float mean[ROWS], rstd[ROWS];
        bool live[ROWS];
#pragma unroll
        for (int rr = 0; rr < ROWS; ++rr) {
            live[rr] = row0 + rr < M;
            const float* xr = x + (size_t)min(row0 + rr, M - 1) * H;
#pragma unroll
            for (int j = 0; j < NCH; ++j) v[rr][j] = act[j] ? *(const f32x4*)(xr + 4 * (lane + 64 * j)) : (f32x4){0, 0, 0, 0};
        }
#pragma unroll
        for (int rr = 0; rr < ROWS; ++rr) {
            float s = 0.f;
#pragma unroll
            for (int j = 0; j < NCH; ++j) s += (v[rr][j][0] + v[rr][j][1]) + (v[rr][j][2] + v[rr][j][3]);
            mean[rr] = wave_sum(s) * invH;
            float q = 0.f;
#pragma unroll
            for (int j = 0; j < NCH; ++j) {
                if (act[j]) {
#pragma unroll
                    for (int e = 0; e < 4; ++e) {
                        const float d = v[rr][j][e] - mean[rr];
                        q += d * d;
                    }
                }
            }
            const float var = wave_sum(q) * invH;
            rstd[rr] = rsqrtf(var + eps);
            if (stats != nullptr && lane == 0 && live[rr]) *(float2*)(stats + 2 * (size_t)(row0 + rr)) = make_float2(mean[rr], rstd[rr]);
        }
        float tp[ROWS][8];
#pragma unroll
        for (int rr = 0; rr < ROWS; ++rr)
#pragma unroll
            for (int r = 0; r < 8; ++r) tp[rr][r] = 0.f;
#pragma unroll
        for (int j = 0; j < NCH; ++j) {
            if (!act[j]) continue;
            const int c = 4 * (lane + 64 * j);
            float yb[ROWS][4];
#pragma unroll
            for (int rr = 0; rr < ROWS; ++rr) {
                const int row = row0 + rr;
                f32x4 y;
#pragma unroll
                for (int e = 0; e < 4; ++e) y[e] = (v[rr][j][e] - mean[rr]) * rstd[rr] * g[j][e] + b[j][e];
                if (drop_thr16 > 0) {
                    const unsigned base = (unsigned)row * (unsigned)H + (unsigned)c;
                    float f0, f1, f2, f3;
                    drop_pair(drop_seed, base, (unsigned)drop_thr16, drop_scale, f0, f1);
                    drop_pair(drop_seed, base + 2, (unsigned)drop_thr16, drop_scale, f2, f3);
                    y[0] *= f0; y[1] *= f1; y[2] *= f2; y[3] *= f3;
                }
                uint2 pk;
                pk.x = pack2bf(y[0], y[1]);
                pk.y = pack2bf(y[2], y[3]);
                if (live[rr]) {
                    if (y_f32 != nullptr) *(f32x4*)(y_f32 + (size_t)row * H + c) = y;
                    if (y_bf16 != nullptr) *(uint2*)(y_bf16 + (size_t)row * H + c) = pk;
                    if (y_fp8 != nullptr)
                        *(unsigned*)(y_fp8 + (size_t)row * H + c) = pack4fp8(y[0] * fp8_scale, y[1] * fp8_scale, y[2] * fp8_scale, y[3] * fp8_scale);
                }
                yb[rr][0] = bf2f((unsigned short)(pk.x & 0xffff)); yb[rr][1] = bf2f((unsigned short)(pk.x >> 16));
                yb[rr][2] = bf2f((unsigned short)(pk.y & 0xffff)); yb[rr][3] = bf2f((unsigned short)(pk.y >> 16));
            }
            if (LORA) {
#pragma unroll
                for (int r = 0; r < 8; ++r) {
                    const f32x4 a = *(const f32x4*)(a_lds + r * H + c);
#pragma unroll
                    for (int rr = 0; rr < ROWS; ++rr)
                        tp[rr][r] += (yb[rr][0] * a[0] + yb[rr][1] * a[1]) + (yb[rr][2] * a[2] + yb[rr][3] * a[3]);
                }
            }
        }
        if (LORA) {
#pragma unroll
            for (int rr = 0; rr < ROWS; ++rr) {
                const float tv = wave_reduce8(tp[rr], lane);
                if ((lane & 7) == 0 && live[rr]) t_bf16[(size_t)(row0 + rr) * 8 + (lane >> 3)] = f2bf(tv);
            }
        }
    }
}

template <int NCH, bool PG, int ROWS, bool F8>
__device__ __forceinline__ void layernorm_bwd_body(const unsigned short* __restrict__ dy_bf16,
                                                   const float* __restrict__ dy_f32,
                                                   const float* __restrict__ x,
                                                   const float* __restrict__ stats,
                                                   const float* __restrict__ gamma, int M, int H,
                                                   const float* __restrict__ dres,
                                                   float* __restrict__ dx_f32,
                                                   unsigned short* __restrict__ dx_bf16, unsigned drop_seed,
                                                   int drop_thr16, float drop_scale, float* __restrict__ dgamma,
                                                   float* __restrict__ dbeta, const unsigned short* __restrict__ dres_b16,
                                                   unsigned short* __restrict__ dx_res_b16, unsigned char* __restrict__ dx_fp8,
                                                   float* __restrict__ row_dequant, float* __restrict__ pg_ws) {
    const int lane = threadIdx.x & 63;
    const int wave_in_grid = blockIdx.x * 4 + (threadIdx.x >> 6);
    const int nwaves = gridDim.x * 4;
    f32x4 g[NCH];
    f32x4 pgam[PG ? NCH : 1], pbet[PG ? NCH : 1];
    bool act[NCH];
#pragma unroll
    for (int j = 0; j < NCH; ++j) {
        const int c = 4 * (lane + 64 * j);
        act[j] = c < H;
        g[j] = act[j] ? *(const f32x4*)(gamma + c) : (f32x4){0, 0, 0, 0};
        if (PG) { pgam[j] = (f32x4){0, 0, 0, 0}; pbet[j] = (f32x4){0, 0, 0, 0}; }
    }
    const float invH = 1.0f / (float)H;
    for (int row0 = wave_in_grid * ROWS; row0 < M; row0 += nwaves * ROWS) {
        constexpr bool RS16 = F8 && ROWS == 2;
        f32x4 gy[ROWS][NCH], xh[ROWS][NCH], rs[RS16 ? 1 : ROWS][RS16 ? 1 : NCH];
        uint2 rsp[RS16 ? ROWS : 1][RS16 ? NCH : 1];
        float rstd[ROWS], m1[ROWS], m2[ROWS];
        bool live[ROWS];
#pragma unroll
        for (int rr = 0; rr < ROWS; ++rr) {
            live[rr] = row0 + rr < M;
            const size_t row = (size_t)min(row0 + rr, M - 1);
            const float mean = stats[2 * row];
            rstd[rr] = stats[2 * row + 1];
#pragma unroll
            for (int j = 0; j < NCH; ++j) {
                gy[rr][j] = (f32x4){0, 0, 0, 0};
                xh[rr][j] = (f32x4){0, 0, 0, 0};
                if constexpr (RS16) rsp[rr][j] = make_uint2(0u, 0u);
// ... 288 lines not shown
```

clibd_amd/engine.py:

```python
from __future__ import annotations

import math
import os
from dataclasses import dataclass, field
from typing import List, Optional, Sequence

import torch

from . import ops

BF16, F32 = torch.bfloat16, torch.float32


class NotSupportedYet(NotImplementedError):
    pass


NUMERICS_CHOICES = dict(residual_grad=("bf16", "fp32"), gelu_grad=("bf16", "u8", "e4m7"), attn_bwd=("2phase", "sp"), ln_fold=("off", "on"),
                        dgrad=("bf16", "fp8"))
_NUMERICS_ENV = dict(residual_grad="CLIBD_RESIDUAL_GRAD", gelu_grad="CLIBD_GELU_GRAD", attn_bwd="CLIBD_ATTN_BWD", ln_fold="CLIBD_LN_FOLD",
                     dgrad="CLIBD_DGRAD")


def default_deterministic() -> bool:
    return os.environ.get("CLIBD_DETERMINISTIC", "0") == "1"


def _ordered(on: bool) -> dict:
    return {"ordered": True} if on else {}


def default_numerics() -> dict:
    out = {}
    for k, choices in NUMERICS_CHOICES.items():
        v = os.environ.get(_NUMERICS_ENV[k], choices[0]).lower()
        out[k] = v if v in choices else choices[0]
    return out


def check_numerics(settings: dict) -> dict:
    for k, v in settings.items():
        if k not in NUMERICS_CHOICES:
            raise ValueError(f"unknown numerics switch {k!r} (known: {sorted(NUMERICS_CHOICES)})")
        if v not in NUMERICS_CHOICES[k]:
            raise ValueError(f"numerics switch {k}: {v!r} is not one of {NUMERICS_CHOICES[k]}")
    return settings


def _mul_aux_act(h, FF: int) -> int:
    if h.dtype == torch.uint8:
        return ops.ACT_MUL_AUX_E12 if h.shape[1] == 3 * FF // 2 else ops.ACT_MUL_AUX_U8
    return ops.ACT_MUL_AUX


@dataclass
class LoraParams:
    a_q: torch.nn.Parameter
    b_q: torch.nn.Parameter
    a_v: torch.nn.Parameter
    b_v: torch.nn.Parameter

    def tensors(self):
        return [self.a_q, self.b_q, self.a_v, self.b_v]


@dataclass
class LayerSpec:
    qkv_w: Sequence[torch.Tensor]
    qkv_b: Sequence[torch.Tensor]
    proj_w: torch.Tensor
    proj_b: torch.Tensor
    fc1_w: torch.Tensor
    fc1_b: torch.Tensor
    fc2_w: torch.Tensor
    fc2_b: torch.Tensor
    ln1_w: torch.Tensor
    ln1_b: torch.Tensor
    ln2_w: torch.Tensor
    ln2_b: torch.Tensor
    lora: Optional[LoraParams] = None

    def frozen(self):
        return [*self.qkv_w, *self.qkv_b, self.proj_w, self.proj_b, self.fc1_w, self.fc1_b, self.fc2_w, self.fc2_b, self.ln1_w,
                self.ln1_b, self.ln2_w, self.ln2_b]


class _LayerCache:
    __slots__ = ("wqkv", "wqkv_t", "bqkv", "wo", "wo_t", "bo", "w1", "w1_t", "b1", "w2", "w2_t", "b2", "g1", "be1", "g2", "be2",
                 "v_fwd", "v_bwd", "a_cat", "w_dt", "slot2", "wqkv8", "cs_qkv", "wo8", "cs_o", "w18", "cs_1", "w28", "cs_2",
                 "w1g", "s1", "b1f",
                 "wo_t8", "cs_ot", "w1_t8", "cs_1t", "w2_t8", "cs_2t", "c2")


def _f32c(t: torch.Tensor) -> torch.Tensor:
    t = t.detach()
    return t if (t.dtype == F32 and t.is_contiguous()) else t.to(F32).contiguous()


def _rank_slots(lp: "LoraParams"):
    a_q, a_v, b_q, b_v = _f32c(lp.a_q), _f32c(lp.a_v), _f32c(lp.b_q), _f32c(lp.b_v)
    r, H = a_q.shape

    def slot(lo):
        hi = min(lo + 4, r)
        k = hi - lo
        pa = lambda a: a[lo:hi].contiguous() if k == 4 else torch.cat([a[lo:hi], a.new_zeros((4 - k, H))], dim=0)
        pb = lambda b: (b[:, lo:hi] if k == 4 else torch.cat([b[:, lo:hi], b.new_zeros((H, 4 - k))], dim=1)).contiguous()
        return pa(a_q), pa(a_v), pb(b_q), pb(b_v)

    return [slot(lo) for lo in range(0, r, 4)]


class TransformerStack:

    def __init__(self, layers: List[LayerSpec], hidden: int, heads: int, pre_ln: bool, eps: float):
        if hidden != heads * 64:
            raise NotSupportedYet(f"attention kernel is specialised for head_dim 64 (hidden={hidden}, heads={heads})")
        if hidden % 64 or hidden > 1024:
            raise NotSupportedYet("hidden size must be a multiple of 64 and <= 1024")
        self.layers, self.H, self.heads, self.pre_ln, self.eps = layers, hidden, heads, pre_ln, eps
        self.FF = layers[0].fc1_w.shape[0]
        self._cache: List[_LayerCache] = []
        self._cache_key = None
        self.fp8 = None
        self._calib = None
        self.numerics = default_numerics()
        self.deterministic = default_deterministic()
        self._c2, self._c2_age = None, 0
        self.dgrad8_sites = ("mlp", "proj")

    DGRAD8_C2_EVERY = 64

    def set_numerics(self, **settings):
        before = (self.numerics.get("ln_fold"), self.numerics.get("dgrad"))
        self.numerics.update(check_numerics(settings))
        if (self.numerics.get("ln_fold"), self.numerics.get("dgrad")) != before:
            self._cache_key = None
            self._c2 = None

    def _dgrad8_ok(self) -> bool:
        if self.numerics["dgrad"] != "fp8":
            return False
        if self.numerics["residual_grad"] != "bf16":
            raise NotSupportedYet("dgrad=fp8 needs residual_grad=bf16")
        if self.H % 256 or self.H < 512 or self.FF % 256:
            raise NotSupportedYet("dgrad=fp8 needs hidden % 256 == 0, hidden >= 512, intermediate % 256 == 0")
        return True

    FP8_SITES = ("qkv_in", "proj_in", "fc1_in", "fc2_in")
    FP8_SCALES = dict(qkv_in=8.0, proj_in=32.0, fc1_in=8.0, fc2_in=4.0)

    def enable_fp8(self, scales: Optional[dict] = None, amax: Optional[list] = None, margin: float = 2.0, sites: Optional[Sequence[str]] = None):
        if sites is not None:
            sites = tuple(sites)
            if any(s not in self.FP8_SITES for s in sites):
                raise ValueError(f"enable_fp8: sites must come from {self.FP8_SITES}")
            if set(sites) != set(self.FP8_SITES):
                if set(sites) != {"fc1_in", "fc2_in"}:
                    raise NotSupportedYet("fp8 site selection: only the MLP pair (fc1_in, fc2_in) is built")
        if self.full_mode() and (sites is None or set(sites) != {"fc1_in", "fc2_in"}):
            raise NotSupportedYet("fp8 forward on every site needs frozen base weights (their gradients would need the bf16 GEMM inputs); "
                                  "with trainable base weights the MLP-pair selection (sites=('fc1_in', 'fc2_in')) is built")
        if self.H % 256 or self.H < 512 or self.FF % 256:
            raise NotSupportedYet("fp8 forward needs hidden % 256 == 0, hidden >= 512, intermediate % 256 == 0")
        base = dict(self.FP8_SCALES, **(scales or {}))
        if sites is not None:
            base = {k: v for k, v in base.items() if k in sites}
        per_layer = []
        for i in range(len(self.layers)):
            d = dict(base)
            if amax is not None:
                for site, v in amax[i].items():
                    if site not in d:
                        continue
                    v = float(v)
                    if v > 0.0 and math.isfinite(v):
                        d[site] = 2.0 ** math.floor(math.log2(448.0 / (margin * v)))
            per_layer.append(d)
        self.fp8 = per_layer
        self._cache_key = None

    def disable_fp8(self):
        self.fp8 = None
        self._cache_key = None

    def calibrate(self, on: bool = True):
        if on:
            self._calib = []
            return None
        rec, self._calib = self._calib, None
        return [{k: float(v) for k, v in d.items()} for d in (rec or [])]

    def _key(self):
        k = 0
        for L in self.layers:
            for p in L.frozen():
                k += p._version + (p.data_ptr() & 0xFFFF)
        return (k, self.layers[0].proj_w.device)

    def full_mode(self) -> bool:
        return any(p.requires_grad for L in self.layers for p in L.frozen())

    def base_params(self):
        return [p for L in self.layers for p in L.frozen()]

    def refresh(self):
        key = self._key()
        if key == self._cache_key and not self.full_mode():
            return
        self._cache = []
        with torch.no_grad():
            for L in self.layers:
                c = _LayerCache()
                wqkv = _f32c(L.qkv_w[0]) if len(L.qkv_w) == 1 else torch.cat([_f32c(w) for w in L.qkv_w], dim=0)
                c.wqkv, c.wqkv_t = ops.cast_bf16(wqkv), ops.cast_transpose_bf16(wqkv)
                c.bqkv = _f32c(L.qkv_b[0]).clone() if len(L.qkv_b) == 1 else torch.cat([_f32c(b) for b in L.qkv_b], dim=0)
                c.wo, c.wo_t, c.bo = ops.cast_bf16(_f32c(L.proj_w)), ops.cast_transpose_bf16(_f32c(L.proj_w)), _f32c(L.proj_b)
                c.w1, c.w1_t, c.b1 = ops.cast_bf16(_f32c(L.fc1_w)), ops.cast_transpose_bf16(_f32c(L.fc1_w)), _f32c(L.fc1_b)
                c.w2, c.w2_t, c.b2 = ops.cast_bf16(_f32c(L.fc2_w)), ops.cast_transpose_bf16(_f32c(L.fc2_w)), _f32c(L.fc2_b)
                c.g1, c.be1, c.g2, c.be2 = _f32c(L.ln1_w), _f32c(L.ln1_b), _f32c(L.ln2_w), _f32c(L.ln2_b)
                if self.fp8 is not None:
                    f8 = self.fp8[len(self._cache)]
                    if "qkv_in" in f8:
                        c.wqkv8, c.cs_qkv = ops.quantize_rows_fp8(wqkv.contiguous(), f8["qkv_in"])
                        c.wo8, c.cs_o = ops.quantize_rows_fp8(_f32c(L.proj_w), f8["proj_in"])
                    c.w18, c.cs_1 = ops.quantize_rows_fp8(_f32c(L.fc1_w), f8["fc1_in"])
                    c.w28, c.cs_2 = ops.quantize_rows_fp8(_f32c(L.fc2_w), f8["fc2_in"])
                c.w1g = c.s1 = c.b1f = None
                if self.pre_ln and self.numerics["ln_fold"] == "on" and not self.full_mode():
                    c.w1g, c.s1, c.b1f = ops.ln_fold_weights(_f32c(L.fc1_w), c.g2, c.be2, c.b1)
                c.v_fwd = c.v_bwd = c.a_cat = c.w_dt = c.slot2 = None
                c.wo_t8 = c.cs_ot = c.w1_t8 = c.cs_1t = c.w2_t8 = c.cs_2t = c.c2 = None
                self._cache.append(c)
            if self._dgrad8_ok():
                dev = self._cache[0].w2_t.device
                full = self.full_mode()
                reuse = full and self._c2 is not None and len(self._c2) == len(self._cache) and self._c2_age < self.DGRAD8_C2_EVERY
                l1 = None if reuse else torch.zeros((len(self._cache),), dtype=F32, device=dev)
                for i, c in enumerate(self._cache):
                    c.w2_t8, c.cs_2t = ops.quantize_rows_fp8_bf16(c.w2_t, 1.0, None if reuse else l1[i:i + 1])
                    c.wo_t8, c.cs_ot = ops.quantize_rows_fp8_bf16(c.wo_t, 1.0)
                if reuse:
                    self._c2_age += 1
                else:
                    self._c2 = [2.0 ** (math.floor(math.log2(448.0 / (256.0 * 1.13 * max(v, 1e-30)))) - (1 if full else 0))
                                for v in l1.cpu().tolist()]
                    self._c2_age = 1
                for c, c2 in zip(self._cache, self._c2):
                    c.c2 = c2
                    c.w1_t8, c.cs_1t = ops.quantize_rows_fp8_bf16(c.w1_t, c.c2)
        self._cache_key = key

    def pack_lora(self):
        H = self.H
        for L, c in zip(self.layers, self._cache):
            if L.lora is None:
                continue
            dev = L.proj_w.device
            images = lambda: dict(v_fwd=torch.empty((3 * H, 8), dtype=BF16, device=dev), v_bwd=torch.empty((H, 8), dtype=BF16, device=dev),
                                  a_cat=torch.empty((8, H), dtype=BF16, device=dev), w_dt=torch.empty((16, 3 * H), dtype=BF16, device=dev))
            if c.v_fwd is None:
                im = images()
                c.v_fwd, c.v_bwd, c.a_cat, c.w_dt = im["v_fwd"], im["v_bwd"], im["a_cat"], im["w_dt"]
            slots = _rank_slots(L.lora)
            ops.lora_pack(*slots[0], c.v_fwd, c.v_bwd, c.a_cat, c.w_dt)
            if len(slots) > 1:
                if self.fp8 is not None:
                    raise NotSupportedYet("fp8 forward with LoRA rank > 4")
                if c.slot2 is None or len(c.slot2) != len(slots) - 1:
                    c.slot2 = [images() for _ in slots[1:]]
                for sl, im in zip(slots[1:], c.slot2):
                    ops.lora_pack(*sl, im["v_fwd"], im["v_bwd"], im["a_cat"], im["w_dt"])
            else:
                c.slot2 = None

    def _slot2_addend(self, u, v, N, residual=None):
        M = u.shape[0]
        out = torch.empty((M, N), dtype=F32, device=u.device)
        ops.gemm_nt(torch.zeros((M, 64), dtype=BF16, device=u.device), torch.zeros((N, 64), dtype=BF16, device=u.device), rank_u=u, rank_v=v,
                    residual=residual, out_f32=out)
        return out

    def _slot2_fwd(self, c, x_bf16):
        add32, ts = None, []
        for im in c.slot2:
            tj = ops.lora_down_proj(x_bf16, im["a_cat"])
            add32 = self._slot2_addend(tj, im["v_fwd"], 3 * self.H, residual=add32)
            ts.append(tj)
        return add32, ts

    def _slot2_bwd_addend(self, c, dt2, residual=None):
        add32 = residual
        for im, dtj in zip(c.slot2, dt2):
            add32 = self._slot2_addend(dtj, im["v_bwd"], self.H, residual=add32)
        return add32

    def lora_a(self, i: int):
        if i >= len(self.layers) or self.layers[i].lora is None:
            return None
        return self._cache[i].a_cat

    def forward(self, x_f32, x_bf16, t0, B: int, S: int, key_mask, save: bool, cls_only_last: bool = False, drop=None, full: bool = False,
                x_fp8=None):
        H, FF, M = self.H, self.FF, B * S
        dev = x_f32.device
        saved = []
        new = lambda cols, dt: torch.empty((M, cols), dtype=dt, device=dev)
        keep = save and full
        f8s = self.fp8
        mlp_only = f8s is not None and "qkv_in" not in f8s[0]
        if f8s is not None and full and not mlp_only:
            raise NotSupportedYet("fp8 forward on every site with trainable base weights (the MLP-pair selection is built)")
        cal = self._calib if f8s is None else None
        amax = lambda t_: t_.abs().amax().float()
        f8 = None
        AT = ops.FP8 if f8s is not None else BF16
        o = None if keep else new(H, BF16 if mlp_only else AT)
        a = None if keep else new(FF, AT)
        xn2 = new(H, AT) if (self.pre_ln and not keep) else None
        xn8 = new(H, ops.FP8) if (f8s is not None and not mlp_only) else None
        gg = self.numerics["gelu_grad"]
        if f8s is not None or (self.pre_ln and self.numerics["ln_fold"] == "on"):
            gg = "bf16"
        GG = BF16 if gg == "bf16" else torch.uint8
        HC = 3 * FF // 2 if gg == "e4m7" else FF
        act_save = {"bf16": ops.ACT_GELU_SAVE_GRAD, "u8": ops.ACT_GELU_SAVE_GRAD_U8, "e4m7": ops.ACT_GELU_SAVE_GRAD_E12}[gg]
        h_tmp = new(FF, BF16) if (f8s is not None and not save) else None
        t = t0
        sp_ok = save and key_mask is None and f8s is None and S <= 224 and self.numerics["attn_bwd"] == "sp"
        fold = (self.pre_ln and self.numerics["ln_fold"] == "on" and self._cache[0].w1g is not None and f8s is None and not full and GG == BF16 and H % 256 == 0 and FF % 256 == 0
                and M >= 1024 and ((M + 255) // 256) * (H // 256) >= 128 and H % 128 == 0)
        fold_sums = torch.empty((H // 128, M, 2), dtype=F32, device=dev) if fold else None
        if fold and h_tmp is None and not save:
            h_tmp = new(FF, BF16)
        for i, (L, c) in enumerate(zip(self.layers, self._cache)):
            has_lora = L.lora is not None
            rec = {}
            att_sv = None
            t2 = None
            f8 = f8s[i] if f8s is not None else None
            crec = {} if cal is not None else None
            if keep:
                o, a = new(H, BF16), new(FF, AT)
                xn2 = new(H, AT) if self.pre_ln else None
            if self.pre_ln and cls_only_last and i == len(self.layers) - 1:
                xn = new(H, BF16)
                st1 = torch.empty((M, 2), dtype=F32, device=dev)
                t = torch.empty((M, 8), dtype=BF16, device=dev) if has_lora else None
                qkv = new(3 * H, BF16)
                if f8 is not None and not mlp_only:
                    ops.layernorm_fwd(x_f32, c.g1, c.be1, self.eps, y_bf16=xn, stats=st1, lora_a=c.a_cat if has_lora else None, t_out=t,
                                      y_fp8=xn8, fp8_scale=f8["qkv_in"])
                    ops.gemm_fp8_nt(xn8, c.wqkv8, c.cs_qkv, bias=c.bqkv, rank_u=t, rank_v=c.v_fwd if has_lora else None, out_bf16=qkv)
                else:
                    ops.layernorm_fwd(x_f32, c.g1, c.be1, self.eps, y_bf16=xn, stats=st1, lora_a=c.a_cat if has_lora else None, t_out=t)
                    add32, t2 = self._slot2_fwd(c, xn) if c.slot2 is not None else (None, None)
                    ops.gemm_nt(xn, c.wqkv, bias=c.bqkv, rank_u=t, rank_v=c.v_fwd if has_lora else None, residual=add32, out_bf16=qkv)
                    if crec is not None:
                        crec["qkv_in"] = amax(xn)
                newB = lambda cols, dt: torch.empty((B, cols), dtype=dt, device=dev)
                o_cls = newB(H, BF16)
                ops.attention_fwd(qkv, B, S, self.heads, key_mask, o_cls, nq=1)
                x_cls = ops.gather_rows(x_f32.view(B, S, H))
                x1 = newB(H, F32)
                ops.gemm_nt(o_cls, c.wo, bias=c.bo, residual=x_cls, out_f32=x1)
                st2 = torch.empty((B, 2), dtype=F32, device=dev)
                xn2c = newB(H, BF16)
                ops.layernorm_fwd(x1, c.g2, c.be2, self.eps, y_bf16=xn2c, stats=st2)
                h = newB(HC, GG) if save else None
                ac = newB(FF, BF16)
                ops.gemm_nt(xn2c, c.w1, bias=c.b1, act=act_save if save else ops.ACT_GELU, out_pre=h, out_bf16=ac)
                x2 = newB(H, F32)
                ops.gemm_nt(ac, c.w2, bias=c.b2, residual=x1, out_f32=x2)
                if save:
                    rec = dict(x_in=x_f32, st1=st1, xn=xn, t=t, t2=t2, qkv=qkv, x1=x1, st2=st2, h=h, cls_only=True)
                    if keep:
                        rec.update(o=o_cls, xn2=xn2c, a=ac)
                x_f32 = x2
            elif self.pre_ln:
                xn = new(H, BF16)
                st1 = torch.empty((M, 2), dtype=F32, device=dev)
                t = torch.empty((M, 8), dtype=BF16, device=dev) if has_lora else None
                qkv = new(3 * H, BF16)
                x1 = new(H, F32)
                st2 = torch.empty((M, 2), dtype=F32, device=dev)
                h = new(HC, GG) if save else None
                x2 = new(H, F32)
                if f8 is not None and mlp_only:
                    ops.layernorm_fwd(x_f32, c.g1, c.be1, self.eps, y_bf16=xn, stats=st1, lora_a=c.a_cat if has_lora else None, t_out=t)
                    add32, t2 = self._slot2_fwd(c, xn) if c.slot2 is not None else (None, None)
                    ops.gemm_nt(xn, c.wqkv, bias=c.bqkv, rank_u=t, rank_v=c.v_fwd if has_lora else None, residual=add32, out_bf16=qkv)
                    ops.attention_fwd(qkv, B, S, self.heads, key_mask, o)
                    ops.gemm_nt(o, c.wo, bias=c.bo, residual=x_f32, out_f32=x1)
                    ops.layernorm_fwd(x1, c.g2, c.be2, self.eps, stats=st2, y_fp8=xn2, fp8_scale=f8["fc1_in"])
                    ops.gemm_fp8_nt(xn2, c.w18, c.cs_1, bias=c.b1, gelu_out_fp8=a, gelu_out_scale=f8["fc2_in"], out_pre=h if save else h_tmp)
                    ops.gemm_fp8_nt(a, c.w28, c.cs_2, bias=c.b2, residual=x1, out_f32=x2)
                elif f8 is not None:
                    ops.layernorm_fwd(x_f32, c.g1, c.be1, self.eps, y_bf16=xn, stats=st1, lora_a=c.a_cat if has_lora else None, t_out=t,
                                      y_fp8=xn8, fp8_scale=f8["qkv_in"])
                    ops.gemm_fp8_nt(xn8, c.wqkv8, c.cs_qkv, bias=c.bqkv, rank_u=t, rank_v=c.v_fwd if has_lora else None, out_bf16=qkv)
                    ops.attention_fwd(qkv, B, S, self.heads, key_mask, o, out_fp8_scale=f8["proj_in"])
                    ops.gemm_fp8_nt(o, c.wo8, c.cs_o, bias=c.bo, residual=x_f32, out_f32=x1)
                    ops.layernorm_fwd(x1, c.g2, c.be2, self.eps, stats=st2, y_fp8=xn2, fp8_scale=f8["fc1_in"])
                    ops.gemm_fp8_nt(xn2, c.w18, c.cs_1, bias=c.b1, gelu_out_fp8=a, gelu_out_scale=f8["fc2_in"], out_pre=h if save else h_tmp)
                    ops.gemm_fp8_nt(a, c.w28, c.cs_2, bias=c.b2, residual=x1, out_f32=x2)
                else:
                    ops.layernorm_fwd(x_f32, c.g1, c.be1, self.eps, y_bf16=xn, stats=st1, lora_a=c.a_cat if has_lora else None, t_out=t)
                    add32, t2 = self._slot2_fwd(c, xn) if c.slot2 is not None else (None, None)
                    ops.gemm_nt(xn, c.wqkv, bias=c.bqkv, rank_u=t, rank_v=c.v_fwd if has_lora else None, residual=add32, out_bf16=qkv)
                    if sp_ok:
                        o = o if keep else new(H, BF16)
                        att_sv = dict(o_att=o, o_lo=new(H, BF16), lse=torch.empty((B * self.heads * S,), dtype=F32, device=dev))
                        ops.attention_fwd(qkv, B, S, self.heads, None, o, lse=att_sv["lse"], o_lo=att_sv["o_lo"])
                    else:
                        ops.attention_fwd(qkv, B, S, self.heads, key_mask, o)
                    if fold and cal is None:
                        ops.gemm_nt(o, c.wo, bias=c.bo, residual=x_f32, out_f32=x1, out_bf16=xn2, row_sums=fold_sums)
                        ops.rowsum_finalize(fold_sums, self.eps, st2)
                        ops.gemm_nt(xn2, c.w1g, bias=c.b1f, act=ops.ACT_GELU_SAVE_GRAD, out_pre=h if save else h_tmp, out_bf16=a, row_stats=st2, col_sum_w=c.s1)
                    else:
                        ops.gemm_nt(o, c.wo, bias=c.bo, residual=x_f32, out_f32=x1)
                        ops.layernorm_fwd(x1, c.g2, c.be2, self.eps, y_bf16=xn2, stats=st2)
                        ops.gemm_nt(xn2, c.w1, bias=c.b1, act=act_save if save else ops.ACT_GELU, out_pre=h if save else None, out_bf16=a)
                    ops.gemm_nt(a, c.w2, bias=c.b2, residual=x1, out_f32=x2)
                    if crec is not None:
                        crec.update(qkv_in=amax(xn), proj_in=amax(o), fc1_in=amax(xn2), fc2_in=amax(a))
                if save:
                    rec = dict(x_in=x_f32, st1=st1, xn=xn, t=t, t2=t2, qkv=qkv, x1=x1, st2=st2, h=h)
                    if keep:
                        rec.update(o=o, xn2=xn2, a=a)
                        if f8 is not None:
                            rec.update(xn2_s=f8["fc1_in"], a_s=f8["fc2_in"])
                    if att_sv is not None:
                        rec.update(att_sv)
                x_f32 = x2
            else:
                d_att = d_h1 = d_h2 = None
                if drop is not None:
                    p_h, p_a, base = drop
                    d_att = ops.Drop(p_a, ops.derive_seed(base, i, 0))
                    d_h1 = ops.Drop(p_h, ops.derive_seed(base, i, 1))
                    d_h2 = ops.Drop(p_h, ops.derive_seed(base, i, 2))
                qkv = new(3 * H, BF16)
                s1 = new(H, F32)
                x1_f32 = new(H, F32)
                st1 = torch.empty((M, 2), dtype=F32, device=dev)
                h = new(HC, GG) if save else None
                s2 = new(H, F32)
                x2_f32, x2_bf16 = new(H, F32), new(H, BF16)
                st2 = torch.empty((M, 2), dtype=F32, device=dev)
                nxt = self.lora_a(i + 1)
                t_next = torch.empty((M, 8), dtype=BF16, device=dev) if nxt is not None else None
                ru, rv = (t if has_lora else None), (c.v_fwd if has_lora else None)
                if f8 is not None and mlp_only:
                    x1_bf16 = None
                    x18 = new(H, ops.FP8)
                    ops.gemm_nt(x_bf16, c.wqkv, bias=c.bqkv, rank_u=ru, rank_v=rv, out_bf16=qkv)
                    ops.attention_fwd(qkv, B, S, self.heads, key_mask, o, drop=d_att)
                    ops.gemm_nt(o, c.wo, bias=c.bo, residual=x_f32, out_f32=s1, drop=d_h1)
                    ops.layernorm_fwd(s1, c.g1, c.be1, self.eps, y_f32=x1_f32, stats=st1, y_fp8=x18, fp8_scale=f8["fc1_in"])
                    ops.gemm_fp8_nt(x18, c.w18, c.cs_1, bias=c.b1, gelu_out_fp8=a, gelu_out_scale=f8["fc2_in"], out_pre=h if save else h_tmp)
                    ops.gemm_fp8_nt(a, c.w28, c.cs_2, bias=c.b2, residual=x1_f32, out_f32=s2, drop=d_h2)
                    ops.layernorm_fwd(s2, c.g2, c.be2, self.eps, y_bf16=x2_bf16, y_f32=x2_f32, stats=st2, lora_a=nxt, t_out=t_next)
                elif f8 is not None:
                    if x_fp8 is None:
                        raise ValueError("fp8 forward (post-LN): the caller passes the e4m3 image of x")
                    x1_bf16 = None
                    x18 = xn8
                    ops.gemm_fp8_nt(x_fp8, c.wqkv8, c.cs_qkv, bias=c.bqkv, rank_u=ru, rank_v=rv, out_bf16=qkv)
                    ops.attention_fwd(qkv, B, S, self.heads, key_mask, o, drop=d_att, out_fp8_scale=f8["proj_in"])
                    ops.gemm_fp8_nt(o, c.wo8, c.cs_o, bias=c.bo, residual=x_f32, out_f32=s1, drop=d_h1)
                    ops.layernorm_fwd(s1, c.g1, c.be1, self.eps, y_f32=x1_f32, stats=st1, y_fp8=x18, fp8_scale=f8["fc1_in"])
                    ops.gemm_fp8_nt(x18, c.w18, c.cs_1, bias=c.b1, gelu_out_fp8=a, gelu_out_scale=f8["fc2_in"], out_pre=h if save else h_tmp)
                    ops.gemm_fp8_nt(a, c.w28, c.cs_2, bias=c.b2, residual=x1_f32, out_f32=s2, drop=d_h2)
                    x8_next = new(H, ops.FP8)
                    ops.layernorm_fwd(s2, c.g2, c.be2, self.eps, y_bf16=x2_bf16, y_f32=x2_f32, stats=st2, lora_a=nxt, t_out=t_next,
                                      y_fp8=x8_next, fp8_scale=f8s[min(i + 1, len(f8s) - 1)]["qkv_in"])
                    x_fp8 = x8_next
                else:
                    x1_bf16 = new(H, BF16)
                    add32, t2 = self._slot2_fwd(c, x_bf16) if c.slot2 is not None else (None, None)
                    ops.gemm_nt(x_bf16, c.wqkv, bias=c.bqkv, rank_u=ru, rank_v=rv, residual=add32, out_bf16=qkv)
                    if sp_ok:
                        o = o if keep else new(H, BF16)
                        att_sv = dict(o_att=o, o_lo=new(H, BF16), lse=torch.empty((B * self.heads * S,), dtype=F32, device=dev))
                        ops.attention_fwd(qkv, B, S, self.heads, None, o, drop=d_att, lse=att_sv["lse"], o_lo=att_sv["o_lo"])
                    else:
                        ops.attention_fwd(qkv, B, S, self.heads, key_mask, o, drop=d_att)
                    ops.gemm_nt(o, c.wo, bias=c.bo, residual=x_f32, out_f32=s1, drop=d_h1)
                    ops.layernorm_fwd(s1, c.g1, c.be1, self.eps, y_bf16=x1_bf16, y_f32=x1_f32, stats=st1)
                    ops.gemm_nt(x1_bf16, c.w1, bias=c.b1, act=act_save if save else ops.ACT_GELU, out_pre=h if save else None, out_bf16=a)
                    ops.gemm_nt(a, c.w2, bias=c.b2, residual=x1_f32, out_f32=s2, drop=d_h2)
                    ops.layernorm_fwd(s2, c.g2, c.be2, self.eps, y_bf16=x2_bf16, y_f32=x2_f32, stats=st2, lora_a=nxt, t_out=t_next)
                    if crec is not None:
                        crec.update(qkv_in=amax(x_bf16), proj_in=amax(o), fc1_in=amax(x1_bf16), fc2_in=amax(a))
                if save:
                    rec = dict(x_bf16=x_bf16, t=t if has_lora else None, t2=t2, qkv=qkv, s1=s1, st1=st1, h=h, s2=s2, st2=st2,
                               d_att=d_att, d_h1=d_h1, d_h2=d_h2)
                    if keep:
                        rec.update(o=o, x1_bf16=x1_bf16, a=a)
                        if f8 is not None:
                            rec.update(x1_bf16=x18, x1_s=f8["fc1_in"], a_s=f8["fc2_in"])
                    if att_sv is not None:
                        rec.update(att_sv)
                x_f32, x_bf16, t = x2_f32, x2_bf16, t_next
            saved.append(rec)
            if cal is not None:
                cal.append(crec)
        return x_f32, x_bf16, saved

    def layer_params(self, i: int):
        L = self.layers[i]
        return L.frozen() + (L.lora.tensors() if L.lora is not None else [])

    def backward(self, dx_f32, dx_bf16, saved, B: int, S: int, key_mask, grads: dict, full: bool = False, on_layer_done=None):
        H, FF, M = self.H, self.FF, B * S
        dev = dx_f32.device
        new = lambda cols, dt: torch.empty((M, cols), dtype=dt, device=dev)
        dh = None
        dtmp = new(H, BF16)
        dqkv = new(3 * H, BF16)
        dt = torch.empty((M, 16), dtype=BF16, device=dev)
        first_lora = min((i for i, L in enumerate(self.layers) if L.lora is not None), default=len(self.layers))
        if full:
            first_lora = -1
        r16 = self.numerics["residual_grad"] == "bf16"
        dg8 = self._dgrad8_ok() and self._cache[0].w2_t8 is not None and M % 4 == 0 and M * FF < 2 ** 32
        new8 = lambda cols: (torch.empty((M, cols), dtype=torch.uint8, device=dev).view(ops.FP8), torch.empty((M,), dtype=F32, device=dev))
        f8kw = lambda pair: dict(dx_fp8=pair[0], row_dequant=pair[1])
        dx8 = None
        det = self.deterministic
        pg = lambda w, b: (dict(dgamma=grads[id(w)].view(-1), dbeta=grads[id(b)].view(-1), **_ordered(det))
                           if full and id(w) in grads else {})
        wg = lambda dy, x, ws, bs, xs=None: linear_wgrad(dy, x, ws, bs, grads, x_scale=xs, **_ordered(det)) if full else None
        for i in range(len(self.layers) - 1, -1, -1):
            L, c, rec = self.layers[i], self._cache[i], saved[i]
            has_lora = L.lora is not None
            dt2 = None
            if i < first_lora:
                break
            if self.pre_ln and rec.get("cls_only"):
                newB = lambda cols, dt: torch.empty((B, cols), dtype=dt, device=dev)
                dhc, dtc = newB(FF, BF16), newB(H, BF16)
                wg(dx_bf16, rec.get("a"), [L.fc2_w], [L.fc2_b])
                ops.gemm_nt(dx_bf16, c.w2_t, act=_mul_aux_act(rec["h"], FF), aux=rec["h"], out_bf16=dhc)
                wg(dhc, rec.get("xn2"), [L.fc1_w], [L.fc1_b])
                ops.gemm_nt(dhc, c.w1_t, out_bf16=dtc)
                dx1_f32, dx1_bf16 = newB(H, F32), newB(H, BF16)
                ops.layernorm_bwd(dtc, rec["x1"], rec["st2"], c.g2, dres=dx_f32, dx_f32=dx1_f32, dx_bf16=dx1_bf16, **pg(L.ln2_w, L.ln2_b))
                wg(dx1_bf16, rec.get("o"), [L.proj_w], [L.proj_b])
                ops.gemm_nt(dx1_bf16, c.wo_t, out_bf16=dtc)
                ops.attention_bwd(rec["qkv"], dtc, B, S, self.heads, key_mask, dqkv, nq=1)
                if has_lora:
                    dt2 = self._lora_grads(L, c, dqkv, rec["xn"], rec["t"], dt, grads, rec.get("t2"))
                wg(dqkv, rec["xn"], L.qkv_w, L.qkv_b)
                if i > first_lora:
                    add32 = None if dt2 is None else self._slot2_bwd_addend(c, dt2)
                    ops.gemm_nt(dqkv, c.wqkv_t, rank_u=dt if has_lora else None, rank_v=c.v_bwd if has_lora else None, residual=add32, out_bf16=dtmp)
                    if r16:
                        dres16, _ = ops.scatter_rows(dx1_f32, S, bf16=True, f32=False)
                        ndx_bf16 = new(H, BF16)
                        ndx_f32 = new(H, F32) if (full and i == 0) else None
                        dx8 = new8(H) if (dg8 and "mlp" in self.dgrad8_sites) else None
                        ops.layernorm_bwd(dtmp, rec["x_in"], rec["st1"], c.g1, dres_bf16=dres16, dx_bf16=ndx_bf16, dx_f32=ndx_f32, **pg(L.ln1_w, L.ln1_b),
                                          **(f8kw(dx8) if dx8 is not None else {}))
                        dx_f32, dx_bf16 = ndx_f32, ndx_bf16
                    else:
                        _, dres_full = ops.scatter_rows(dx1_f32, S, bf16=False, f32=True)
                        ndx_f32, ndx_bf16 = new(H, F32), new(H, BF16)
                        ops.layernorm_bwd(dtmp, rec["x_in"], rec["st1"], c.g1, dres=dres_full, dx_f32=ndx_f32, dx_bf16=ndx_bf16, **pg(L.ln1_w, L.ln1_b))
                        dx_f32, dx_bf16 = ndx_f32, ndx_bf16
            elif self.pre_ln:
                wg(dx_bf16, rec.get("a"), [L.fc2_w], [L.fc2_b], rec.get("a_s"))
                if dg8 and dx8 is not None:
                    dh8 = torch.empty((M, FF), dtype=torch.uint8, device=dev).view(ops.FP8)
                    if full:
# ... 280 lines not shown
```

clibd_amd/ops.py:

```python
from __future__ import annotations

import ctypes as C
import math
import os
from typing import Optional

import torch

from . import _lib
from ._lib import GemmEpilogue, check

ACT_NONE, ACT_GELU, ACT_GELU_GRAD, ACT_GELU_SAVE_GRAD, ACT_MUL_AUX, ACT_ADD_AUX, ACT_GELU_SAVE_GRAD_U8, ACT_MUL_AUX_U8 = 0, 1, 2, 3, 4, 5, 6, 7
ACT_GELU_SAVE_GRAD_E12, ACT_MUL_AUX_E12 = 8, 9
BF16, F32, I64, I32 = torch.bfloat16, torch.float32, torch.int64, torch.int32
FP8 = torch.float8_e4m3fn


def _stream() -> int:
    return torch._C._cuda_getCurrentRawStream(torch._C._cuda_getDevice())


def _p(t: Optional[torch.Tensor]) -> Optional[int]:
    return None if t is None else t.data_ptr()


def _chk(t: torch.Tensor, dtype, name: str, contiguous: bool = True) -> None:
    if not t.is_cuda:
        raise ValueError(f"{name}: expected a device tensor (clibd_amd has no CPU compute path)")
    if t.dtype != dtype:
        raise TypeError(f"{name}: expected {dtype}, got {t.dtype}")
    if contiguous and not t.is_contiguous():
        raise ValueError(f"{name}: expected a contiguous tensor")


def _rowmajor(t: torch.Tensor, name: str) -> int:
    if t.dim() != 2 or t.stride(1) != 1:
        raise ValueError(f"{name}: expected a 2-D tensor with unit inner stride")
    return t.stride(0)


class Drop:
    __slots__ = ("seed", "thr16", "scale")

    def __init__(self, p: float, seed: int):
        self.thr16 = int(round(p * 65536.0))
        if not 0 <= self.thr16 < 65536:
            raise ValueError("dropout p must be in [0, 1)")
        self.seed = seed & 0xFFFFFFFF
        self.scale = 1.0 / (1.0 - self.thr16 / 65536.0)


def _drop_args(drop: Optional[Drop]) -> tuple:
    return (drop.seed, drop.thr16, drop.scale) if (drop is not None and drop.thr16 > 0) else (0, 0, 1.0)


def derive_seed(base: int, layer: int, site: int) -> int:
    x = (base ^ ((layer * 8 + site + 1) * 0x9E3779B1)) & 0xFFFFFFFF
    x ^= x >> 16
    x = (x * 0x7FEB352D) & 0xFFFFFFFF
    x ^= x >> 15
    x = (x * 0x846CA68B) & 0xFFFFFFFF
    x ^= x >> 16
    return x


_STREAMK = os.environ.get("CLIBD_GEMM_STREAMK", "0") == "1"
_TAIL_WS_BYTES = 48 * 1024 * 1024 + 1024

_workspaces: dict = {"tail": {}}
_tail_ws = _workspaces["tail"]


def _workspace(kind: str, nbytes: int, device, zero: bool = False) -> torch.Tensor:
    cache = _workspaces.setdefault(kind, {})
    key = (device, torch.cuda.current_stream(device).cuda_stream)
    ws = cache.get(key)
    if ws is None or ws.numel() < nbytes:
        ws = (torch.zeros if zero else torch.empty)(((max(int(nbytes), 16) + 15) // 16 * 16,), dtype=torch.uint8, device=device)
        cache[key] = ws
    return ws


def _ws_args(ws: Optional[torch.Tensor]) -> tuple:
    return (None, 0) if ws is None else (ws.data_ptr(), ws.numel())


def _not_ordered(what: str):
    from .engine import NotSupportedYet

    return NotSupportedYet(f"deterministic mode: {what} has no fixed-order form")


def gemm_nt(
    a: torch.Tensor,
    w: torch.Tensor,
    *,
    bias: Optional[torch.Tensor] = None,
    rank_u: Optional[torch.Tensor] = None,
    rank_v: Optional[torch.Tensor] = None,
    act: int = ACT_NONE,
    aux: Optional[torch.Tensor] = None,
    residual: Optional[torch.Tensor] = None,
    out_pre: Optional[torch.Tensor] = None,
    out_bf16: Optional[torch.Tensor] = None,
    out_f32: Optional[torch.Tensor] = None,
    split_k: int = 1,
    drop: Optional["Drop"] = None,
    k_hole: Optional[tuple] = None,
    row_sums: Optional[torch.Tensor] = None,
    row_stats: Optional[torch.Tensor] = None,
    col_sum_w: Optional[torch.Tensor] = None,
) -> None:
    _chk(a, BF16, "a", contiguous=False)
    _chk(w, BF16, "w", contiguous=False)
    lda, ldw = _rowmajor(a, "a"), _rowmajor(w, "w")
    M, K = a.shape
    N, K2 = w.shape
    if K != K2:
        raise ValueError(f"gemm_nt: K mismatch {K} vs {K2}")
    ep = GemmEpilogue()
    ep.act = act
    ep.split_k = split_k
    if drop is not None and drop.thr16 > 0:
        ep.drop_seed, ep.drop_thr16, ep.drop_scale, ep.drop_ld = drop.seed, drop.thr16, drop.scale, N
    if bias is not None:
        _chk(bias, F32, "bias")
        if bias.numel() != N:
            raise ValueError("gemm_nt: bias must have N elements")
        ep.bias = bias.data_ptr()
    if rank_u is not None or rank_v is not None:
        _chk(rank_u, BF16, "rank_u", contiguous=False)
        _chk(rank_v, BF16, "rank_v")
        if rank_u.shape[0] != M or rank_u.shape[1] < 8 or tuple(rank_v.shape) != (N, 8):
            raise ValueError("gemm_nt: rank_u must be [M,>=8], rank_v [N,8]")
        ep.rank_u, ep.rank_v, ep.ld_rank_u = rank_u.data_ptr(), rank_v.data_ptr(), _rowmajor(rank_u, "rank_u")
    if aux is not None:
        _chk(aux, torch.uint8 if act in (ACT_MUL_AUX_U8, ACT_MUL_AUX_E12) else BF16, "aux", contiguous=False)
        if tuple(aux.shape) != (M, 3 * N // 2 if act == ACT_MUL_AUX_E12 else N):
            raise ValueError("gemm_nt: aux must be [M,N] ([M,3N/2] bytes for the e4m7 form)")
        ep.aux_bf16, ep.ld_aux = aux.data_ptr(), _rowmajor(aux, "aux")
    if residual is not None:
        _chk(residual, F32, "residual", contiguous=False)
        if tuple(residual.shape) != (M, N):
            raise ValueError("gemm_nt: residual must be [M,N]")
        ep.residual_f32, ep.ld_res = residual.data_ptr(), _rowmajor(residual, "residual")
    for name, t, dt in (("out_pre", out_pre, torch.uint8 if act in (ACT_GELU_SAVE_GRAD_U8, ACT_GELU_SAVE_GRAD_E12) else BF16), ("out_bf16", out_bf16, BF16), ("out_f32", out_f32, F32)):
        if t is not None:
            _chk(t, dt, name, contiguous=False)
            if tuple(t.shape) != (M, 3 * N // 2 if (name == "out_pre" and act == ACT_GELU_SAVE_GRAD_E12) else N):
                raise ValueError(f"gemm_nt: {name} must be [M,N] ([M,3N/2] bytes for the e4m7 form)")
    if out_pre is not None:
        ep.out_pre_bf16, ep.ld_pre = out_pre.data_ptr(), _rowmajor(out_pre, "out_pre")
    if out_bf16 is not None:
        ep.out_bf16, ep.ld_out_bf16 = out_bf16.data_ptr(), _rowmajor(out_bf16, "out_bf16")
    if out_f32 is not None:
        ep.out_f32, ep.ld_out_f32 = out_f32.data_ptr(), _rowmajor(out_f32, "out_f32")
    if row_sums is not None:
        _chk(row_sums, F32, "row_sums")
        if N % 128 or tuple(row_sums.shape) != (N // 128, M, 2):
            raise ValueError("gemm_nt: row_sums must be [N/128, M, 2]")
        ep.row_sums = row_sums.data_ptr()
    if row_stats is not None or col_sum_w is not None:
        _chk(row_stats, F32, "row_stats")
        _chk(col_sum_w, F32, "col_sum_w")
        if tuple(row_stats.shape) != (M, 2) or col_sum_w.numel() != N:
            raise ValueError("gemm_nt: row_stats must be [M,2], col_sum_w [N]")
        ep.row_stats, ep.col_sum_w = row_stats.data_ptr(), col_sum_w.data_ptr()
    if k_hole is not None:
        check(_lib.load().clibd_gemm_bf16_nt_khole(a.data_ptr(), lda, w.data_ptr(), ldw, M, N, K, int(k_hole[0]), int(k_hole[1]), C.byref(ep),
                                                   _stream()), "gemm_bf16_nt_khole")
        return
    lib = _lib.load()
    ws = None
    if _STREAMK and split_k == 1 and M >= 1024:
        need = int(lib.clibd_gemm_tail_workspace_bytes(M, N, K))
        if need > 0:
            ws = _workspace("tail", max(need, _TAIL_WS_BYTES), a.device, zero=True)
    check(lib.clibd_gemm_bf16_nt(a.data_ptr(), lda, w.data_ptr(), ldw, M, N, K, C.byref(ep), *_ws_args(ws), _stream()), "gemm_bf16_nt")


def rowsum_finalize(row_sums: torch.Tensor, eps: float, stats: torch.Tensor) -> None:
    _chk(row_sums, F32, "row_sums")
    _chk(stats, F32, "stats")
    S, M, _ = row_sums.shape
    if tuple(stats.shape) != (M, 2):
        raise ValueError("rowsum_finalize: stats must be [M,2]")
    check(_lib.load().clibd_rowsum_finalize(row_sums.data_ptr(), S, M, 128 * S, float(eps), stats.data_ptr(), _stream()), "rowsum_finalize")


def ln_fold_weights(w: torch.Tensor, gamma: torch.Tensor, beta: torch.Tensor, bias: Optional[torch.Tensor]):
    _chk(w, F32, "w")
    _chk(gamma, F32, "gamma")
    _chk(beta, F32, "beta")
    N, K = w.shape
    wg = torch.empty((N, K), dtype=BF16, device=w.device)
    s = torch.empty((N,), dtype=F32, device=w.device)
    bp = torch.empty((N,), dtype=F32, device=w.device)
    check(_lib.load().clibd_ln_fold_weights(w.data_ptr(), gamma.data_ptr(), beta.data_ptr(), bias.data_ptr() if bias is not None else None, N, K,
                                            wg.data_ptr(), s.data_ptr(), bp.data_ptr(), _stream()), "ln_fold_weights")
    return wg, s, bp


def quantize_rows_fp8(w: torch.Tensor, act_scale: float):
    _chk(w, F32, "w")
    N, K = w.shape
    w8 = torch.empty((N, K), dtype=torch.uint8, device=w.device).view(FP8)
    cs = torch.empty((N,), dtype=F32, device=w.device)
    check(_lib.load().clibd_quantize_rows_fp8(w.data_ptr(), N, K, float(act_scale), w8.data_ptr(), cs.data_ptr(), _stream()), "quantize_rows_fp8")
    return w8, cs


def quantize_rows_fp8_bf16(w: torch.Tensor, act_scale: float = 1.0, l1max: Optional[torch.Tensor] = None):
    _chk(w, BF16, "w")
    N, K = w.shape
    w8 = torch.empty((N, K), dtype=torch.uint8, device=w.device).view(FP8)
    cs = torch.empty((N,), dtype=F32, device=w.device)
    if l1max is not None:
        _chk(l1max, F32, "l1max")
    check(_lib.load().clibd_quantize_rows_fp8_bf16(w.data_ptr(), N, K, float(act_scale), w8.data_ptr(), cs.data_ptr(), _p(l1max), _stream()),
          "quantize_rows_fp8_bf16")
    return w8, cs


def gemm_fp8_dgrad_nt(a: torch.Tensor, w: torch.Tensor, col_scale: torch.Tensor, *, a_row_dequant: Optional[torch.Tensor] = None,
                      aux: Optional[torch.Tensor] = None, act: int = ACT_NONE, out_bf16: Optional[torch.Tensor] = None,
                      out_fp8: Optional[torch.Tensor] = None, out_fp8_scale: float = 0.0, out_bf16_dual: Optional[torch.Tensor] = None) -> None:
    _chk(a, FP8, "a", contiguous=False)
    _chk(w, FP8, "w", contiguous=False)
    _chk(col_scale, F32, "col_scale")
    lda, ldw = _rowmajor(a, "a"), _rowmajor(w, "w")
    M, K = a.shape
    N, K2 = w.shape
    if K != K2 or col_scale.numel() != N:
        raise ValueError("gemm_fp8_dgrad_nt: shape mismatch")
    if act not in (ACT_NONE, ACT_ADD_AUX, ACT_MUL_AUX, ACT_MUL_AUX_U8, ACT_MUL_AUX_E12):
        raise ValueError("gemm_fp8_dgrad_nt: act must be NONE, ADD_AUX, MUL_AUX, MUL_AUX_U8 or MUL_AUX_E12")
    if (act == ACT_NONE) != (aux is None):
        raise ValueError("gemm_fp8_dgrad_nt: aux comes with ADD_AUX / MUL_AUX only")
    ep = GemmEpilogue()
    ep.split_k = 1
    ep.act = act
    if aux is not None:
        _chk(aux, torch.uint8 if act in (ACT_MUL_AUX_U8, ACT_MUL_AUX_E12) else BF16, "aux", contiguous=False)
        if tuple(aux.shape) != (M, 3 * N // 2 if act == ACT_MUL_AUX_E12 else N):
            raise ValueError("gemm_fp8_dgrad_nt: aux must be [M,N] ([M,3N/2] bytes for the e4m7 form)")
        ep.aux_bf16, ep.ld_aux = aux.data_ptr(), _rowmajor(aux, "aux")
    if act in (ACT_MUL_AUX, ACT_MUL_AUX_U8, ACT_MUL_AUX_E12):
        if out_fp8 is None or out_bf16 is not None or not out_fp8_scale > 0:
            raise ValueError("gemm_fp8_dgrad_nt: the MUL_AUX form writes out_fp8 with a positive out_fp8_scale")
        _chk(out_fp8, FP8, "out_fp8", contiguous=False)
# ... 820 lines not shown
```

include/clibd_hip.h:

```cpp
#ifndef CLIBD_HIP_H
#define CLIBD_HIP_H
#include <stddef.h>
#include <stdint.h>

#ifdef __cplusplus
extern "C" {
#endif

#define CLIBD_OK 0
#define CLIBD_EINVAL (-1)
#define CLIBD_ELAUNCH (-2)

const char* clibd_last_error(void);
int clibd_abi_version(void);
const char* clibd_build_hash(void);

enum { CLIBD_ACT_NONE = 0, CLIBD_ACT_GELU = 1, CLIBD_ACT_GELU_GRAD = 2, CLIBD_ACT_GELU_SAVE_GRAD = 3, CLIBD_ACT_MUL_AUX = 4,
       CLIBD_ACT_ADD_AUX = 5, CLIBD_ACT_GELU_SAVE_GRAD_U8 = 6, CLIBD_ACT_MUL_AUX_U8 = 7,
       CLIBD_ACT_GELU_SAVE_GRAD_E12 = 8, CLIBD_ACT_MUL_AUX_E12 = 9  };

typedef struct clibd_gemm_epilogue {
    const float* bias;
    const void* rank_u;
    const void* rank_v;
    const void* aux_bf16;
    const float* residual_f32;
    void* out_pre_bf16;
    void* out_bf16;
    float* out_f32;
    int32_t act;
    int32_t ld_rank_u, ld_aux, ld_res, ld_pre, ld_out_bf16, ld_out_f32;
    int32_t split_k;
    uint32_t drop_seed;
    int32_t drop_thr16;
    float drop_scale;
    int32_t drop_ld;
    float* row_sums;
    const float* row_stats;
    const float* col_sum_w;
} clibd_gemm_epilogue;

size_t clibd_gemm_tail_workspace_bytes(int M, int N, int K);
int clibd_gemm_bf16_nt(const void* A, int lda, const void* W, int ldw, int M, int N, int K,
                       const clibd_gemm_epilogue* ep, void* workspace, size_t workspace_bytes, void* stream);
int clibd_gemm_bf16_nt_khole(const void* A, int lda, const void* W, int ldw, int M, int N, int K, int hole_k0, int hole_len,
                             const clibd_gemm_epilogue* ep, void* stream);

int clibd_gemm_fp8_nt(const void* A, int lda, const void* W, int ldw, int M, int N, int K, const float* col_scale,
                      float out_fp8_scale, const clibd_gemm_epilogue* ep, void* stream);

int clibd_quantize_rows_fp8(const float* w, int N, int K, float act_scale, void* w_fp8, float* col_scale, void* stream);

int clibd_gemm_fp8_dgrad_nt(const void* A, int lda, const void* W, int ldw, int M, int N, int K, const float* col_scale,
                            const float* a_row_dequant, float out_fp8_scale, const clibd_gemm_epilogue* ep, void* stream);
int clibd_quantize_rows_fp8_bf16(const void* w_bf16, int N, int K, float act_scale, void* w_fp8, float* col_scale, float* l1max, void* stream);

int clibd_transpose_bf16(const void* in, int ld_in, int R, int C, void* out, int ld_out, void* stream);
int clibd_transpose_fp8_bf16(const void* in, int ld_in, int R, int C, float scale, void* out, int ld_out, void* stream);
size_t clibd_transpose_colsum_workspace_bytes(int ld_out, int C);
int clibd_transpose_colsum_bf16(const void* in, int ld_in, int R, int C, void* out, int ld_out, float* colsum, void* workspace,
                                size_t workspace_bytes, void* stream);

int clibd_cast_f32_to_bf16(const float* in, void* out, size_t n, void* stream);
int clibd_cast_transpose_f32_to_bf16(const float* in, int R, int C, void* out, void* stream);

int clibd_layernorm_fwd(const float* x, int M, int H, const float* gamma, const float* beta, float eps,
                        void* y_bf16, float* y_f32, float* stats, const void* lora_a_bf16, void* t_bf16,
                        uint32_t drop_seed, int drop_thr16, float drop_scale, void* y_fp8, float fp8_scale, void* stream);
size_t clibd_layernorm_bwd_pg_workspace_bytes(int M, int H);
int clibd_layernorm_bwd(const void* dy_bf16, const float* dy_f32, const float* x, const float* stats, const float* gamma, int M, int H,
                        const float* dres_f32, const void* dres_bf16, float* dx_f32, void* dx_res_bf16, void* dx_bf16,
                        uint32_t drop_seed, int drop_thr16, float drop_scale, void* dx_fp8, float* row_dequant,
                        float* dgamma, float* dbeta, void* workspace, size_t workspace_bytes, void* stream);

int clibd_attention_fwd(const void* qkv, int B, int S, int nheads, const int32_t* key_mask, void* out, int nq, int out_seq,
                        uint32_t drop_seed, int drop_thr16, float drop_scale, float out_fp8_scale, float* lse, void* o_lo,
                        void* stream);
int clibd_attention_bwd(const void* qkv, const void* dout, int B, int S, int nheads, const int32_t* key_mask, void* dqkv,
                        int nq, int dout_seq, uint32_t drop_seed, int drop_thr16, float drop_scale, void* stream);

int clibd_attention_bwd_sp(const void* qkv, const void* dout, const void* out, const void* o_lo, const float* lse, int B, int S,
                           int nheads, void* dqkv, uint32_t drop_seed, int drop_thr16, float drop_scale, void* stream);

int clibd_lora_pack(const float* a_q, const float* a_v, const float* b_q, const float* b_v, int H,
                    void* v_fwd_bf16, void* v_bwd_bf16, void* a_cat_bf16, void* w_dt_bf16, void* stream);
int clibd_lora_down_proj(const void* x_bf16, int ld_x, const void* a_cat_bf16, int M, int H, void* t_bf16, void* stream);
size_t clibd_lora_workspace_bytes(int M, int H);
int clibd_lora_wgrad(const void* dqkv, int ld_dqkv, const void* x_bf16, const void* t_bf16, const void* dt_bf16,
                     int ld_dt, int M, int H, float* dA_q, float* dA_v, float* dB_q, float* dB_v,
                     void* workspace, size_t workspace_bytes, void* stream);
int clibd_lora_backward(const void* dqkv, int ld_dqkv, const void* x_bf16, const void* t_bf16, const void* w_dt_bf16,
                        void* dt_bf16, int ld_dt, int M, int H, float* dA_q, float* dA_v, float* dB_q, float* dB_v,
                        void* workspace, size_t workspace_bytes, void* stream);

int clibd_patchify(const float* image, int B, void* patches_bf16, void* stream);
int clibd_patchify_u8(const unsigned char* image, int B, void* patches_bf16, void* stream);
int clibd_rowsum_finalize(const float* row_sums, int slices, int M, int H, float eps, float* stats, void* stream);
int clibd_ln_fold_weights(const float* w, const float* gamma, const float* beta, const float* bias, int N, int K, void* wg_bf16,
                          float* col_sum_w, float* bias_folded, void* stream);
int clibd_vit_assemble_tokens(const float* proj, const float* cls, const float* pos, int B, int S, int H, float* tok,
                              void* stream);
int clibd_bert_embed(const int64_t* ids, const int64_t* token_type, int B, int S, int H, int vocab,
// ... 94 lines not shown
```

Baseline: 7131.

## Recompute post-LN residual inside GEMM epilogue instead of storing f32 LN output

```diff
diff --git a/clibd_amd/csrc/common.h b/clibd_amd/csrc/common.h
--- a/clibd_amd/csrc/common.h
+++ b/clibd_amd/csrc/common.h
@@ -66,6 +66,12 @@
 __device__ __forceinline__ float drop_one(unsigned seed, unsigned idx, unsigned thr16, float scale) {
     const unsigned h = drop_hash(seed, idx >> 1);
     return (((idx & 1u) ? (h >> 16) : (h & 0xffffu)) >= thr16) ? scale : 0.f;
+}
+
+__device__ __forceinline__ float ln_affine(float x, float mean, float rstd, float g, float b) {
+    const float d = x - mean;
+    const float t = d * rstd;
+    return __builtin_fmaf(t, g, b);
 }
 
 template <int CTRL>
diff --git a/clibd_amd/csrc/gemm.hip b/clibd_amd/csrc/gemm.hip
--- a/clibd_amd/csrc/gemm.hip
+++ b/clibd_amd/csrc/gemm.hip
@@ -131,7 +131,7 @@
         for (int j = 0; j < 4; ++j)
 #pragma unroll
             for (int r = 0; r < 4; ++r) v[4 * j + r] = acc[i][j][r] + bias[4 * j + r];
-        store_row16(ep, m, nb, v);
+        store_row16(ep, m, nb, p.N, v);
     }
 }
 
@@ -333,7 +333,16 @@
         return set_error(CLIBD_EINVAL, "gemm: GELU_SAVE_GRAD_E12 needs out_pre (1.5 bytes per element) with ld_pre >= 3N/2 bytes, % 4");
     if ((ep->act == CLIBD_ACT_GELU_SAVE_GRAD || ep->act == CLIBD_ACT_GELU_SAVE_GRAD_U8) && !ep->out_pre_bf16)
         return set_error(CLIBD_EINVAL, "gemm: GELU_SAVE_GRAD needs out_pre_bf16");
-    if (ep->act < 0 || ep->act > CLIBD_ACT_MUL_AUX_E12) return set_error(CLIBD_EINVAL, "gemm: bad act");
+    if (ep->act < 0 || ep->act > CLIBD_ACT_RESIDUAL_LN) return set_error(CLIBD_EINVAL, "gemm: bad act");
+    const bool res_ln = ep->act == CLIBD_ACT_RESIDUAL_LN;
+    if (res_ln) {
+        if (!ep->residual_f32 || !ep->row_stats || !ep->col_sum_w || !ep->out_f32)
+            return set_error(CLIBD_EINVAL, "gemm: RESIDUAL_LN needs residual_f32 (the pre-LN sum), row_stats (mean, rstd per row), col_sum_w (gamma || beta) and out_f32");
+        if (ep->out_bf16 || ep->out_pre_bf16 || ep->rank_u || ep->rank_v || ep->row_sums || ep->aux_bf16 || ep->split_k > 1)
+            return set_error(CLIBD_EINVAL, "gemm: RESIDUAL_LN takes no out_bf16, out_pre_bf16, rank update, row_sums, aux or split-K");
+        if (!aligned16(ep->col_sum_w) || ((uintptr_t)ep->row_stats & 7))
+            return set_error(CLIBD_EINVAL, "gemm: RESIDUAL_LN: col_sum_w must be 16-byte aligned, row_stats 8-byte aligned");
+    }
     if (ep->residual_f32 && (ep->ld_res % 4 || ep->ld_res < N)) return set_error(CLIBD_EINVAL, "gemm: ld_res");
     if (ep->out_pre_bf16 && (ep->ld_pre % (ep->act == CLIBD_ACT_GELU_SAVE_GRAD_U8 ? 16 : 8) || ep->ld_pre < N)) return set_error(CLIBD_EINVAL, "gemm: ld_pre");
     if (ep->out_bf16 && (ep->ld_out_bf16 % 8 || ep->ld_out_bf16 < N)) return set_error(CLIBD_EINVAL, "gemm: ld_out_bf16");
@@ -367,7 +376,7 @@
         p.sk_ws = (float*)((char*)tail_ws + 1024);
     }
     static const int forced = [] { const char* e = getenv("CLIBD_GEMM_KERNEL"); return e ? atoi(e) : 0; }();
-    const bool fold_epi = ep->row_sums != nullptr || ep->row_stats != nullptr;
+    const bool fold_epi = !res_ln && (ep->row_sums != nullptr || ep->row_stats != nullptr);
     if (fold_epi) {
         if (epilogue_kind(p.ep) < 0)
             return set_error(CLIBD_EINVAL, "gemm: LN-fold epilogue: row_sums needs bias + residual_f32 + out_f32 + out_bf16 (act NONE); row_stats needs "
diff --git a/clibd_amd/csrc/gemm256.hip b/clibd_amd/csrc/gemm256.hip
--- a/clibd_amd/csrc/gemm256.hip
+++ b/clibd_amd/csrc/gemm256.hip
@@ -374,13 +374,15 @@
         asm volatile("" : "+v"(erow), "+v"(egrp));
         int nb = n0 + 128 * wm + 8 * erow;
         int mb = m0 + 64 * wn + 4 * egrp;
-        constexpr bool RES_KIND = (KIND == EPI_RES_F32 || KIND == EPI_RES_F32_DROP || KIND == EPI_RES_F32_COPY);
+        constexpr bool RES_LN = epi_res_ln_kind(KIND);
+        constexpr bool RES_KIND = (KIND == EPI_RES_F32 || KIND == EPI_RES_F32_DROP || KIND == EPI_RES_F32_COPY || RES_LN);
         constexpr bool TWO_PASS = (epi_aux_kind(KIND) || RES_KIND || KIND == EPI_ROWNORM_GELU);
         constexpr bool PRELOAD_ROWS = TWO_PASS && !LORA && !FP8;
         f32x4 bias_q[2];
         uint4 in_aux[8];
         f32x4 in_res[8][2];
         float2 in_st[8];
+        f32x4 ln_gb[4];
         f32x4 col_s[2];
 #define GLOAD128(dst, ptr) asm volatile("global_load_dwordx4 %0, %1, off ; EPI_OPERAND_LOAD" : "=&v"(dst) : "v"(ptr) : "memory")
         constexpr bool BIAS_ASM = BIAS && !FP8;
@@ -391,12 +393,12 @@
         }
         if constexpr (PRELOAD_ROWS) {
 #pragma unroll
-            for (int n = 0; n < 2; ++n)
+            for (int n = 0; n < (RES_LN ? 1 : 2); ++n)
 #pragma unroll
                 for (int r = 0; r < 4; ++r) {
                     const int mc = min(mb + 16 * n + r, p.M - 1);
+                    if constexpr (KIND == EPI_ROWNORM_GELU || RES_LN) in_st[4 * n + r] = *(const float2*)(ep.row_stats + (size_t)mc * 2);
                     if constexpr (KIND == EPI_ROWNORM_GELU) {
-                        in_st[4 * n + r] = *(const float2*)(ep.row_stats + (size_t)mc * 2);
                     } else if constexpr (KIND == EPI_MUL_AUX_U8) {
                         const uint2 c8 = *(const uint2*)((const unsigned char*)ep.aux_bf16 + (size_t)mc * ep.ld_aux + nb);
                         in_aux[4 * n + r] = make_uint4(c8.x, c8.y, 0u, 0u);
@@ -415,6 +417,13 @@
             col_s[0] = *(const f32x4*)(ep.col_sum_w + nb);
             col_s[1] = *(const f32x4*)(ep.col_sum_w + nb + 4);
         }
+        if constexpr (RES_LN) {
+            static_assert(PRELOAD_ROWS, "the RESIDUAL_LN kinds are instantiated without LoRA / fp8");
+            ln_gb[0] = *(const f32x4*)(ep.col_sum_w + nb);
+            ln_gb[1] = *(const f32x4*)(ep.col_sum_w + nb + 4);
+            ln_gb[2] = *(const f32x4*)(ep.col_sum_w + p.N + nb);
+            ln_gb[3] = *(const f32x4*)(ep.col_sum_w + p.N + nb + 4);
+        }
         if (has_next) {
             ISSUE(1, 2, 1); __builtin_amdgcn_sched_barrier(0);
             ISSUE(1, 3, 1); __builtin_amdgcn_sched_barrier(0);
@@ -430,6 +439,9 @@
         if constexpr (KIND == EPI_ROWNORM_GELU) {
             if (!has_next) asm volatile("s_waitcnt vmcnt(10)" ::: "memory");
             EPI_TIED_WAIT(14);
+        } else if constexpr (RES_LN) {
+            if (!has_next) asm volatile("s_waitcnt vmcnt(16)" ::: "memory");
+            EPI_TIED_WAIT(20);
         } else if constexpr (PRELOAD_ROWS && epi_aux_kind(KIND)) {
             if (!has_next) asm volatile("s_waitcnt vmcnt(8)" ::: "memory");
             EPI_TIED_WAIT(12);
@@ -544,7 +556,38 @@
                 if constexpr (KIND == EPI_ROWNORM_GELU) {
                     _Pragma("unroll") for (int e = 0; e < 4; ++e) { cs8[e] = col_s[0][e]; cs8[4 + e] = col_s[1][e]; }
                 }
-                FOR_ROWS_HN(0, 1, {
+                if constexpr (RES_LN) {
+                    _Pragma("unroll") for (int hn = 0; hn < 2; ++hn)
+                        _Pragma("unroll") for (int n = 0; n < 2; ++n) {
+                            if (hn + n > 0) {
+                                _Pragma("unroll") for (int r = 0; r < 4; ++r)
+                                    in_st[r] = *(const float2*)(ep.row_stats + (size_t)min(mb + 32 * hn + 16 * n + r, p.M - 1) * 2);
+                                _Pragma("unroll") for (int r = 0; r < 4; ++r) {
+                                    const int mc = min(mb + 32 * hn + 16 * n + r, p.M - 1);
+                                    const f32x4* rs = (const f32x4*)(ep.residual_f32 + (size_t)mc * ep.ld_res + nb);
+                                    in_res[r][0] = rs[0];
+                                    in_res[r][1] = rs[1];
+                                }
+                                _Pragma("unroll") for (int r = 0; r < 4; ++r) asm volatile("" : "+v"(in_st[r].x), "+v"(in_st[r].y));
+                                __builtin_amdgcn_sched_barrier(0);
+                            }
+                            _Pragma("unroll") for (int r = 0; r < 4; ++r) {
+                                const int mc = min(mb + 32 * hn + 16 * n + r, p.M - 1);
+                                float v[8];
+                                _Pragma("unroll") for (int hm = 0; hm < 2; ++hm)
+                                    _Pragma("unroll") for (int t = 0; t < 4; ++t) v[4 * hm + t] = EPV(hm, t);
+                                ln_residual4(in_res[r][0], in_st[r].x, in_st[r].y, ln_gb[0], ln_gb[2]);
+                                ln_residual4(in_res[r][1], in_st[r].x, in_st[r].y, ln_gb[1], ln_gb[3]);
+                                fold_row8_in<KIND>(ep, mc, nb, v, make_uint4(0u, 0u, 0u, 0u), in_res[r][0], in_res[r][1]);
+                                _Pragma("unroll") for (int hm = 0; hm < 2; ++hm)
+                                    _Pragma("unroll") for (int t = 0; t < 4; ++t) acc[hm][t][hn][n][r] = v[4 * hm + t];
+                            }
+                            _Pragma("unroll") for (int hm = 0; hm < 2; ++hm)
+                                _Pragma("unroll") for (int t = 0; t < 4; ++t) asm volatile("" : "+v"(acc[hm][t][hn][n]));
+                            __builtin_amdgcn_sched_barrier(0);
+                        }
+                }
+                FOR_ROWS_HN(0, RES_LN ? 0 : 1, {
                     const int mc = min(m, p.M - 1);
                     float v[8];
                     _Pragma("unroll") for (int hm = 0; hm < 2; ++hm)
@@ -555,8 +598,8 @@
                     _Pragma("unroll") for (int hm = 0; hm < 2; ++hm)
                         _Pragma("unroll") for (int t = 0; t < 4; ++t) acc[hm][t][hn][n][r] = v[4 * hm + t];
                 })
-                PIN_GROUP(0);
-                FOR_ROWS_HN(1, 2, {
+                if constexpr (!RES_LN) PIN_GROUP(0);
+                FOR_ROWS_HN(RES_LN ? 2 : 1, 2, {
                     const int mc = min(m, p.M - 1);
                     float v[8];
                     _Pragma("unroll") for (int hm = 0; hm < 2; ++hm)
@@ -570,7 +613,7 @@
                     _Pragma("unroll") for (int hm = 0; hm < 2; ++hm)
                         _Pragma("unroll") for (int t = 0; t < 4; ++t) acc[hm][t][hn][n][r] = v[4 * hm + t];
                 })
-                PIN_GROUP(1);
+                if constexpr (!RES_LN) PIN_GROUP(1);
                 float keep1 = 0.f, keep2 = 0.f;
                 FOR_ROWS({
                     if (m < p.M) {
@@ -697,6 +740,8 @@
         case EPI_SPLITK_F32: return (const void*)gemm256_bf16_nt_kernel<EPI_SPLITK_F32, false, false, false, false>;
         case EPI_RES_F32_COPY: return (lora || !bias || diag) ? nullptr : (const void*)gemm256_bf16_nt_kernel<EPI_RES_F32_COPY, false, true, false, false>;
         case EPI_ROWNORM_GELU: return (lora || !bias || diag) ? nullptr : (const void*)gemm256_bf16_nt_kernel<EPI_ROWNORM_GELU, false, true, false, false>;
+        case EPI_RES_LN_F32: return (lora || !bias || diag) ? nullptr : (const void*)gemm256_bf16_nt_kernel<EPI_RES_LN_F32, false, true, false, false>;
+        case EPI_RES_LN_F32_DROP: return (lora || !bias || diag) ? nullptr : (const void*)gemm256_bf16_nt_kernel<EPI_RES_LN_F32_DROP, false, true, false, false>;
         default: return K256(EPI_GENERIC);
     }
 #undef K256
diff --git a/clibd_amd/csrc/gemm_common.h b/clibd_amd/csrc/gemm_common.h
--- a/clibd_amd/csrc/gemm_common.h
+++ b/clibd_amd/csrc/gemm_common.h
@@ -83,7 +83,12 @@
     }
 }
 
-__device__ __forceinline__ void store_row16(const clibd_gemm_epilogue& ep, int m, int nb, float v[16]) {
+__device__ __forceinline__ void ln_residual4(f32x4& r, float mean, float rstd, const f32x4& g, const f32x4& b) {
+#pragma unroll
+    for (int e = 0; e < 4; ++e) r[e] = ln_affine(r[e], mean, rstd, g[e], b[e]);
+}
+
+__device__ __forceinline__ void store_row16(const clibd_gemm_epilogue& ep, int m, int nb, int N, float v[16]) {
     if (ep.split_k > 1) {
         float* o = ep.out_f32 + (size_t)m * ep.ld_out_f32 + nb;
 #pragma unroll
@@ -174,9 +179,12 @@
     }
     if (ep.residual_f32 != nullptr) {
         const f32x4* rs = (const f32x4*)(ep.residual_f32 + (size_t)m * ep.ld_res + nb);
+        const bool ln = ep.act == CLIBD_ACT_RESIDUAL_LN;
+        const float2 st = ln ? *(const float2*)(ep.row_stats + (size_t)m * 2) : make_float2(0.f, 1.f);
 #pragma unroll
         for (int q = 0; q < 4; ++q) {
-            const f32x4 r4 = rs[q];
+            f32x4 r4 = rs[q];
+            if (ln) ln_residual4(r4, st.x, st.y, *(const f32x4*)(ep.col_sum_w + nb + 4 * q), *(const f32x4*)(ep.col_sum_w + N + nb + 4 * q));
             v[4 * q + 0] += r4[0]; v[4 * q + 1] += r4[1]; v[4 * q + 2] += r4[2]; v[4 * q + 3] += r4[3];
         }
     }
@@ -227,14 +235,20 @@
     EPI_MUL_AUX_12 = 13,
     EPI_GELU = 14,
     EPI_F32 = 15,
-    EPI_NUM_KINDS = 16,
+    EPI_RES_LN_F32 = 16,
+    EPI_RES_LN_F32_DROP = 17,
+    EPI_NUM_KINDS = 18,
 };
+constexpr bool epi_res_ln_kind(int kind) { return kind == EPI_RES_LN_F32 || kind == EPI_RES_LN_F32_DROP; }
 constexpr bool epi_aux_kind(int kind) { return kind == EPI_MUL_AUX || kind == EPI_ADD_AUX || kind == EPI_MUL_AUX_U8 || kind == EPI_MUL_AUX_12; }
 constexpr bool epi_mul_aux_kind(int kind) { return kind == EPI_MUL_AUX || kind == EPI_MUL_AUX_U8 || kind == EPI_MUL_AUX_12; }
 
 __host__ __device__ inline int epilogue_kind(const clibd_gemm_epilogue& ep) {
     if (ep.split_k > 1) return EPI_GENERIC;
     const bool drop = ep.drop_thr16 > 0;
+    if (ep.act == CLIBD_ACT_RESIDUAL_LN)
+        return (!ep.out_pre_bf16 && ep.residual_f32 && ep.row_stats && ep.col_sum_w && !ep.row_sums && ep.out_f32 && !ep.out_bf16 && !ep.rank_u && ep.bias)
+                   ? (drop ? EPI_RES_LN_F32_DROP : EPI_RES_LN_F32) : -1;
     if (ep.row_sums != nullptr)
         return (ep.act == CLIBD_ACT_NONE && !drop && !ep.out_pre_bf16 && ep.residual_f32 && ep.out_f32 && ep.out_bf16 && !ep.rank_u && ep.bias) ? EPI_RES_F32_COPY : -1;
     if (ep.row_stats != nullptr)
@@ -423,7 +437,7 @@
             else { v[2 * e] += a0; v[2 * e + 1] += a1; }
         }
     } else {
-        if (KIND == EPI_RES_F32_DROP) {
+        if (KIND == EPI_RES_F32_DROP || KIND == EPI_RES_LN_F32_DROP) {
             const unsigned base = (unsigned)m * (unsigned)ep.drop_ld + (unsigned)nb;
 #pragma unroll
             for (int e = 0; e < 8; e += 2) {
@@ -495,6 +509,16 @@
     fold_row8_in<KIND>(ep, m, nb, v, ax, r0, r1);
 }
 
+template <int KIND>
+__device__ __forceinline__ void fold_row8_ln(const clibd_gemm_epilogue& ep, int m, int nb, float v[8], const f32x4 gb[4]) {
+    const f32x4* rs = (const f32x4*)(ep.residual_f32 + (size_t)m * ep.ld_res + nb);
+    f32x4 r0 = rs[0], r1 = rs[1];
+    const float2 st = *(const float2*)(ep.row_stats + (size_t)m * 2);
+    ln_residual4(r0, st.x, st.y, gb[0], gb[2]);
+    ln_residual4(r1, st.x, st.y, gb[1], gb[3]);
+    fold_row8_in<KIND>(ep, m, nb, v, make_uint4(0u, 0u, 0u, 0u), r0, r1);
+}
+
 inline int plan_k_slices(int nk, int tiles, int num_cus, int* nks_out) {
     int splits = num_cus / (tiles > 0 ? tiles : 1);
     if (splits < 1) splits = 1;
diff --git a/clibd_amd/csrc/layernorm.hip b/clibd_amd/csrc/layernorm.hip
--- a/clibd_amd/csrc/layernorm.hip
+++ b/clibd_amd/csrc/layernorm.hip
@@ -105,7 +105,7 @@
                 const int row = row0 + rr;
                 f32x4 y;
 #pragma unroll
-                for (int e = 0; e < 4; ++e) y[e] = (v[rr][j][e] - mean[rr]) * rstd[rr] * g[j][e] + b[j][e];
+                for (int e = 0; e < 4; ++e) y[e] = ln_affine(v[rr][j][e], mean[rr], rstd[rr], g[j][e], b[j][e]);
                 if (drop_thr16 > 0) {
                     const unsigned base = (unsigned)row * (unsigned)H + (unsigned)c;
                     float f0, f1, f2, f3;
diff --git a/clibd_amd/engine.py b/clibd_amd/engine.py
--- a/clibd_amd/engine.py
+++ b/clibd_amd/engine.py
@@ -89,7 +89,11 @@
     __slots__ = ("wqkv", "wqkv_t", "bqkv", "wo", "wo_t", "bo", "w1", "w1_t", "b1", "w2", "w2_t", "b2", "g1", "be1", "g2", "be2",
                  "v_fwd", "v_bwd", "a_cat", "w_dt", "slot2", "wqkv8", "cs_qkv", "wo8", "cs_o", "w18", "cs_1", "w28", "cs_2",
                  "w1g", "s1", "b1f",
+                 "gb1", "gb2",
                  "wo_t8", "cs_ot", "w1_t8", "cs_1t", "w2_t8", "cs_2t", "c2")
+
+
+RESIDUAL_LN = True
 
 
 def _f32c(t: torch.Tensor) -> torch.Tensor:
@@ -219,6 +223,9 @@
                 c.w1, c.w1_t, c.b1 = ops.cast_bf16(_f32c(L.fc1_w)), ops.cast_transpose_bf16(_f32c(L.fc1_w)), _f32c(L.fc1_b)
                 c.w2, c.w2_t, c.b2 = ops.cast_bf16(_f32c(L.fc2_w)), ops.cast_transpose_bf16(_f32c(L.fc2_w)), _f32c(L.fc2_b)
                 c.g1, c.be1, c.g2, c.be2 = _f32c(L.ln1_w), _f32c(L.ln1_b), _f32c(L.ln2_w), _f32c(L.ln2_b)
+                c.gb1 = c.gb2 = None
+                if not self.pre_ln:
+                    c.gb1, c.gb2 = torch.cat([c.g1.reshape(-1), c.be1.reshape(-1)]), torch.cat([c.g2.reshape(-1), c.be2.reshape(-1)])
                 if self.fp8 is not None:
                     f8 = self.fp8[len(self._cache)]
                     if "qkv_in" in f8:
@@ -333,6 +340,7 @@
         fold_sums = torch.empty((H // 128, M, 2), dtype=F32, device=dev) if fold else None
         if fold and h_tmp is None and not save:
             h_tmp = new(FF, BF16)
+        x_ln = None
         for i, (L, c) in enumerate(zip(self.layers, self._cache)):
             has_lora = L.lora is not None
             rec = {}
@@ -441,13 +449,15 @@
                     d_att = ops.Drop(p_a, ops.derive_seed(base, i, 0))
                     d_h1 = ops.Drop(p_h, ops.derive_seed(base, i, 1))
                     d_h2 = ops.Drop(p_h, ops.derive_seed(base, i, 2))
+                res_ln = RESIDUAL_LN and f8 is None
+                last = i == len(self.layers) - 1
                 qkv = new(3 * H, BF16)
                 s1 = new(H, F32)
-                x1_f32 = new(H, F32)
+                x1_f32 = None if res_ln else new(H, F32)
                 st1 = torch.empty((M, 2), dtype=F32, device=dev)
                 h = new(HC, GG) if save else None
                 s2 = new(H, F32)
-                x2_f32, x2_bf16 = new(H, F32), new(H, BF16)
+                x2_f32, x2_bf16 = (None if (res_ln and not last) else new(H, F32)), new(H, BF16)
                 st2 = torch.empty((M, 2), dtype=F32, device=dev)
                 nxt = self.lora_a(i + 1)
                 t_next = torch.empty((M, 8), dtype=BF16, device=dev) if nxt is not None else None
@@ -487,11 +497,13 @@
                         ops.attention_fwd(qkv, B, S, self.heads, None, o, drop=d_att, lse=att_sv["lse"], o_lo=att_sv["o_lo"])
                     else:
                         ops.attention_fwd(qkv, B, S, self.heads, key_mask, o, drop=d_att)
-                    ops.gemm_nt(o, c.wo, bias=c.bo, residual=x_f32, out_f32=s1, drop=d_h1)
+                    ops.gemm_nt(o, c.wo, bias=c.bo, residual=x_f32 if x_ln is None else x_ln[0], residual_ln=None if x_ln is None else x_ln[1:],
+                                out_f32=s1, drop=d_h1)
                     ops.layernorm_fwd(s1, c.g1, c.be1, self.eps, y_bf16=x1_bf16, y_f32=x1_f32, stats=st1)
                     ops.gemm_nt(x1_bf16, c.w1, bias=c.b1, act=act_save if save else ops.ACT_GELU, out_pre=h if save else None, out_bf16=a)
-                    ops.gemm_nt(a, c.w2, bias=c.b2, residual=x1_f32, out_f32=s2, drop=d_h2)
+                    ops.gemm_nt(a, c.w2, bias=c.b2, residual=s1 if res_ln else x1_f32, residual_ln=(st1, c.gb1) if res_ln else None, out_f32=s2, drop=d_h2)
                     ops.layernorm_fwd(s2, c.g2, c.be2, self.eps, y_bf16=x2_bf16, y_f32=x2_f32, stats=st2, lora_a=nxt, t_out=t_next)
+                    x_ln = (s2, st2, c.gb2) if x2_f32 is None else None
                     if crec is not None:
                         crec.update(qkv_in=amax(x_bf16), proj_in=amax(o), fc1_in=amax(x1_bf16), fc2_in=amax(a))
                 if save:
diff --git a/clibd_amd/ops.py b/clibd_amd/ops.py
--- a/clibd_amd/ops.py
+++ b/clibd_amd/ops.py
@@ -12,6 +12,7 @@
 
 ACT_NONE, ACT_GELU, ACT_GELU_GRAD, ACT_GELU_SAVE_GRAD, ACT_MUL_AUX, ACT_ADD_AUX, ACT_GELU_SAVE_GRAD_U8, ACT_MUL_AUX_U8 = 0, 1, 2, 3, 4, 5, 6, 7
 ACT_GELU_SAVE_GRAD_E12, ACT_MUL_AUX_E12 = 8, 9
+ACT_RESIDUAL_LN = 10
 BF16, F32, I64, I32 = torch.bfloat16, torch.float32, torch.int64, torch.int32
 FP8 = torch.float8_e4m3fn
 
@@ -110,6 +111,7 @@
     row_sums: Optional[torch.Tensor] = None,
     row_stats: Optional[torch.Tensor] = None,
     col_sum_w: Optional[torch.Tensor] = None,
+    residual_ln: Optional[tuple] = None,
 ) -> None:
     _chk(a, BF16, "a", contiguous=False)
     _chk(w, BF16, "w", contiguous=False)
@@ -166,6 +168,15 @@
         if tuple(row_stats.shape) != (M, 2) or col_sum_w.numel() != N:
             raise ValueError("gemm_nt: row_stats must be [M,2], col_sum_w [N]")
         ep.row_stats, ep.col_sum_w = row_stats.data_ptr(), col_sum_w.data_ptr()
+    if residual_ln is not None:
+        stats, gamma_beta = residual_ln
+        if act != ACT_NONE or residual is None or row_stats is not None or col_sum_w is not None:
+            raise ValueError("gemm_nt: residual_ln goes with residual, act NONE and no fold operands")
+        _chk(stats, F32, "residual_ln stats")
+        _chk(gamma_beta, F32, "residual_ln gamma_beta")
+        if tuple(stats.shape) != (M, 2) or gamma_beta.numel() != 2 * N:
+            raise ValueError("gemm_nt: residual_ln = (stats [M,2], gamma || beta [2N])")
+        ep.act, ep.row_stats, ep.col_sum_w = ACT_RESIDUAL_LN, stats.data_ptr(), gamma_beta.data_ptr()
     if k_hole is not None:
         check(_lib.load().clibd_gemm_bf16_nt_khole(a.data_ptr(), lda, w.data_ptr(), ldw, M, N, K, int(k_hole[0]), int(k_hole[1]), C.byref(ep),
                                                    _stream()), "gemm_bf16_nt_khole")
diff --git a/include/clibd_hip.h b/include/clibd_hip.h
--- a/include/clibd_hip.h
+++ b/include/clibd_hip.h
@@ -17,7 +17,8 @@
 
 enum { CLIBD_ACT_NONE = 0, CLIBD_ACT_GELU = 1, CLIBD_ACT_GELU_GRAD = 2, CLIBD_ACT_GELU_SAVE_GRAD = 3, CLIBD_ACT_MUL_AUX = 4,
        CLIBD_ACT_ADD_AUX = 5, CLIBD_ACT_GELU_SAVE_GRAD_U8 = 6, CLIBD_ACT_MUL_AUX_U8 = 7,
-       CLIBD_ACT_GELU_SAVE_GRAD_E12 = 8, CLIBD_ACT_MUL_AUX_E12 = 9  };
+       CLIBD_ACT_GELU_SAVE_GRAD_E12 = 8, CLIBD_ACT_MUL_AUX_E12 = 9 ,
+       CLIBD_ACT_RESIDUAL_LN = 10  };
 
 typedef struct clibd_gemm_epilogue {
     const float* bias;
```

Result: no change. 7171, median of 6 (+0.6%).
